# facebookresearch/robust-dynrf

Hardware: AMD Instinct MI355X
Metric: training rays/sec (Nvidia Balloon1, configs/Nvidia.txt, static+dynamic TensorVMSplit) (higher is better)
Workload: dtype f32; 1 GPU; BASELINE.json configs[1]: Nvidia Balloon1, configs/Nvidia.txt, 4096 rays/iter/GPU, 1xMI355X per rank, static+dynamic TensorVMSplit; one step = 5 dynamic + 5 static forward passes, scene-flow MLP, induced flow/disparity, per-frame depth loss, distortion loss, compositor, factor regularisers, full backward, Adam; config=nvidia, stage=stage0, samples_per_ray=115, global_batch=4096, rays_per_gpu=4096, parallelism=ray-sharded dp1, ranks=1, dead_work=executed (work the reference also computes although nothing consumes it)

## Files before the change

robust-dynrf_amd/csrc/rdrf_bwd.hip:

```cpp
#ifdef RDRF_GROWS_TEMPORAL
#define RDRF_SAVE_TEMPORAL
#endif
#include "rdrf_kernels.hpp"
#ifdef RDRF_NO_BIAS_ATOMICS
#define BIAS_ATOMIC(p, v) ((void)0)
#else
#define BIAS_ATOMIC(p, v) grad_add(p, v)
#endif

namespace pkb {
constexpr int K1H_DEN2 = 0;
constexpr int K1H_BLE2 = K1H_DEN2 + 64;
#ifdef RDRF_HEADS_BWD_F32
constexpr int K1H_DEN1T_F = K1H_BLE2 + 64;
constexpr int K1H_DEN1T_X0 = K1H_DEN1T_F + 3 * 32 * 64;
constexpr int K1H_BLE1T_F = K1H_DEN1T_X0 + 2 * 32 * 64;
constexpr int K1H_BLE1T_X0 = K1H_BLE1T_F + 3 * 32 * 64;
constexpr int K1H_SIZE = K1H_BLE1T_X0 + 2 * 32 * 64;
#else
constexpr int K1H_DEN1T_F = K1H_BLE2 + 64;
constexpr int K1H_DEN1T_X0 = K1H_DEN1T_F + 3 * 32 * 96;
constexpr int K1H_BLE1T_F = K1H_DEN1T_X0 + 2 * 32 * 96;
constexpr int K1H_BLE1T_X0 = K1H_BLE1T_F + 3 * 32 * 96;
constexpr int K1H_SIZE = K1H_BLE1T_X0 + 2 * 32 * 96;
#endif
constexpr int K1W_W5 = 0;
#ifdef RDRF_HEADS_BWD_F32
constexpr int K1W_W4T = K1W_W5 + 3 * 64;
constexpr int K1W_W3T_X0 = K1W_W4T + 2 * 32 * 64;
constexpr int K1W_W3T_T = K1W_W3T_X0 + 2 * 32 * 64;
constexpr int K1W_SIZE = K1W_W3T_T + 1 * 32 * 64;
#else
constexpr int K1W_W4T = K1W_W5 + 3 * 64;
constexpr int K1W_W3T_X0 = K1W_W4T + 2 * 32 * 96;
constexpr int K1W_W3T_T = K1W_W3T_X0 + 2 * 32 * 96;
constexpr int K1W_SIZE = K1W_W3T_T + 1 * 32 * 96;
#endif
constexpr int K3_RGBV = 0;
constexpr int K3_RGB2T = K3_RGBV + 3 * 128;
constexpr int K3_RGB1T_F = K3_RGB2T + 4 * 64 * 64;
constexpr int K3_RGB1T_X0 = K3_RGB1T_F + 1 * 64 * 64;
constexpr int K3_BASIST = K3_RGB1T_X0 + 2 * 64 * 64;
constexpr int K3_SIZE = K3_BASIST + 7 * 16 * 64;
constexpr int S3_W3 = 0;
constexpr int S3_W2T = S3_W3 + 3 * 128;
constexpr int S3_W1T_F = S3_W2T + 4 * 64 * 64;
constexpr int S3_W1T_P = S3_W1T_F + 1 * 64 * 64;
constexpr int S3_BASIST = S3_W1T_P + 4 * 64 * 64;
constexpr int S3_SIZE = S3_BASIST + 3 * 16 * 64;
constexpr int SF_W6 = 0;
constexpr int SF_W4T = SF_W6 + 6 * 64;
constexpr int SF_W2T = SF_W4T + 2 * 32 * 64;
constexpr int SF_W0T = SF_W2T + 2 * 32 * 64;
constexpr int SF_SIZE = SF_W0T + 2 * 32 * 64;
constexpr int REG_K1H = 0, REG_K1W = REG_K1H + K1H_SIZE, REG_K3 = REG_K1W + K1W_SIZE,
              REG_SF = REG_K3 + K3_SIZE, REG_DYN_END = REG_SF + SF_SIZE;
constexpr int REG_S3 = 0, REG_STAT_END = S3_SIZE;
constexpr int K3_LO_RGB2T = 0;
constexpr int K3_LO_RGB1T = K3_LO_RGB2T + 4 * 64 * 32;
constexpr int K3_LO_BASIST = K3_LO_RGB1T + 3 * 64 * 32;
constexpr int K3_LO_SIZE = K3_LO_BASIST + 7 * 16 * 32;
constexpr int S3_LO_W2T = 0;
constexpr int S3_LO_W1T = S3_LO_W2T + 4 * 64 * 32;
constexpr int S3_LO_BASIST = S3_LO_W1T + 5 * 64 * 32;
constexpr int S3_LO_SIZE = S3_LO_BASIST + 3 * 16 * 32;
constexpr int REG_K3_LO = REG_DYN_END, REG_S3_LO = REG_STAT_END;
static_assert(K3_RGB1T_X0 == K3_RGB1T_F + 64 * 64 && S3_W1T_P == S3_W1T_F + 64 * 64, "layer-1 blocks form one image");
static_assert(K1H_SIZE * 4 <= 160 * 1024 && K3_SIZE * 4 <= 160 * 1024 && S3_SIZE * 4 <= 160 * 1024,
              "backward weight images must fit the LDS");
}


#define DFS_FLOATS 144
RDRF_HD constexpr int dfs_off(int Q) {
  return (Q % 6) < 4 ? (Q / 6) * 16 + 4 * (Q % 6) : ((Q % 6) == 4 ? 48 + 4 * (Q / 6) : 60 + 4 * (Q / 6));
}

#define DFA_FLOATS 216
RDRF_HD constexpr int dfa_off(int Q) {
  return (Q % 18) < 12 ? (Q / 18) * 48 + 4 * (Q % 18)
                       : ((Q % 18) < 15 ? 144 + 12 * (Q / 18) + 4 * ((Q % 18) - 12) : 180 + 12 * (Q / 18) + 4 * ((Q % 18) - 15));
}

struct BwdArgs {
  const float* rays;
  const float* ts;
  const float* xyz;
  const float* z;
  const uint8_t* valid;
  int N, S;
  Box box;
  float distance_scale, weight_thres, density_shift;
  int act, ray_type, static_head;
  const float *g_rgb, *g_sigma, *g_weight, *g_dists, *g_blending, *g_xyz_prime;
  SavedPtrs sp;
  const float* pk;
  float* grows1;
  float* grows3;
  float* dxw_app;
  float* dxn_app;
  float* dtout;
  float* dfs;
  float* dfa;
  float* g_xyz;
  float* g_rays;
  float* g_z;
  int M, in_norm;
  const float* g_feat;
  int small_dw;
  int dynq;
};

struct StaticG {
  RdrfVM density, app;
  float *b3, *w3;
};
struct DynG {
  RdrfVM density, blending, app;
  float *rbv, *rwv, *l5b, *db2, *bb2;
  float *l5w, *dw2, *bw2;
};

template <int CTRL, int ROW_MASK = 0xF>
RDRF_D float dppf(float v) {
  if constexpr (ROW_MASK == 0xF)
    return __int_as_float(__builtin_amdgcn_update_dpp(0, __float_as_int(v), CTRL, 0xF, 0xF, true));
  else
    return __int_as_float(__builtin_amdgcn_update_dpp(__float_as_int(v), __float_as_int(v), CTRL, ROW_MASK, 0xF, false));
}
template <int CTRL, int ROW_MASK = 0xF>
RDRF_D int dppi(int v) {
  if constexpr (ROW_MASK == 0xF)
    return __builtin_amdgcn_update_dpp(0, v, CTRL, 0xF, 0xF, true);
  else
    return __builtin_amdgcn_update_dpp(v, v, CTRL, ROW_MASK, 0xF, false);
}

template <int K>
RDRF_D void atomic_quad_k(float* base, unsigned off, float val, int c) {
  constexpr int QP = K * 0x55;
  const unsigned o = (unsigned)dppi<QP>((int)off);
  if (__ballot(o != 0xffffffffu) == 0ull) return;
  if (o != 0xffffffffu) grad_add(base + (size_t)o + c, val);
}
RDRF_D void atomic_add4(float* p_base, size_t p_off, f32x4 v, bool ok) {
#if defined(RDRF_ABL_NOATOM) || defined(RDRF_ABL_NOGLOBAL)
  return;
#endif
  if (__ballot(ok) == 0ull) return;
  const int lane = threadIdx.x, c = lane & 3;
  const bool a = lane & 1, b = lane & 2;
  const float px = dppf<0xB1>(v.x), py = dppf<0xB1>(v.y), pz = dppf<0xB1>(v.z), pw = dppf<0xB1>(v.w);
  const float n0 = a ? py : v.x, n1 = a ? v.y : px, n2 = a ? pw : v.z, n3 = a ? v.w : pz;
  const float q0 = dppf<0x4E>(n0), q1 = dppf<0x4E>(n1), q2 = dppf<0x4E>(n2), q3 = dppf<0x4E>(n3);
  const float t0 = b ? q2 : n0, t1 = b ? q3 : n1, t2 = b ? n2 : q0, t3 = b ? n3 : q1;
  const unsigned off = ok ? (unsigned)p_off : 0xffffffffu;
  atomic_quad_k<0>(p_base, off, t0, c);
  atomic_quad_k<1>(p_base, off, t1, c);
  atomic_quad_k<2>(p_base, off, t2, c);
  atomic_quad_k<3>(p_base, off, t3, c);
}
RDRF_D float dot4(f32x4 a, f32x4 b) { return a.x * b.x + a.y * b.y + a.z * b.z + a.w * b.w; }

struct Run {
  int start;
  bool tail;
};
RDRF_D Run run_of(int key, int s) {
  const int prev = dppi<0x138>(key);
  const bool head = (s == 0) || (prev != key);
  const unsigned long long b = __ballot(head);
  const unsigned m = (unsigned)(b >> (32 * ((threadIdx.x & 63) >> 5)));
  Run r;
  r.start = 31 - __clz((int)(m & (0xffffffffu >> (31 - s))));
  r.tail = (s == 31) || ((m >> (s + 1)) & 1u);
  return r;
}
RDRF_D f32x4 run_scan4(f32x4 v, int start, int s) {
#ifdef RDRF_ABL_NOSCAN
  return v;
#endif
  const int sr = s & 15;
#define RDRF_SCAN_STEP(D)                                                                   \
  {                                                                                         \
// ... 768 lines not shown
  const int lane = threadIdx.x;
  const int n = blockIdx.x;
  if (n >= a.N) return;
  float vx, vy, vz;
  const float nrm = ray_norm(a.rays, n, a.ray_type, vx, vy, vz);
  if (a.g_weight) {
    float carry = 1.0f;
    for (int j0 = 0; j0 < a.S; j0 += 64) {
      if (lane == 0) carr[j0 >> 6] = carry;
      const int j = j0 + lane;
      const bool act = j < a.S;
      const int idx = n * a.S + (act ? j : 0);
      const bool vld = act && a.valid[idx] != 0;
      const float sigma = vld ? density_act(a.sp.raw[idx], a.act, a.density_shift) : 0.f;
      const float zj = act ? a.z[idx] : 0.f;
      const float zn = (j + 1 < a.S) ? a.z[idx + 1] : zj;
      const float ds = ((j + 1 < a.S) ? (zn - zj) : 0.0f) * nrm * a.distance_scale;
      const float alpha = 1.0f - expf(-sigma * ds);
      const float p = act ? one_minus_alpha_eps(alpha) : 1.0f;
      carry *= __shfl(scan_mul64(p, lane), 63, 64);
    }
  }
  __syncthreads();
  float sufcarry = 0.f, g_nrm = 0.f;
  const int ntile = (a.S + 63) >> 6;
  for (int tl = ntile - 1; tl >= 0; --tl) {
    const int j0 = tl << 6;
    const int j = j0 + lane;
    const bool act = j < a.S;
    const int idx = n * a.S + (act ? j : 0);
    const bool vld = act && a.valid[idx] != 0;
    const float f = a.sp.raw[idx];
    const float sigma = vld ? density_act(f, a.act, a.density_shift) : 0.f;
    const float zj = act ? a.z[idx] : 0.f;
    const float zn = (j + 1 < a.S) ? a.z[idx + 1] : zj;
    const float ds = ((j + 1 < a.S) ? (zn - zj) : 0.0f) * nrm * a.distance_scale;
    const float alpha = 1.0f - expf(-sigma * ds);
    const float p = act ? one_minus_alpha_eps(alpha) : 1.0f;
    float g_alpha = 0.f;
    if (a.g_weight) {
      const float incl = scan_mul64(p, lane);
      float excl = __shfl_up(incl, 1, 64);
      if (lane == 0) excl = 1.0f;
      const float T = carr[tl] * excl;
      const float gwv = act ? a.g_weight[idx] : 0.f;
      float rinc = gwv * alpha * T;
#pragma unroll
      for (int d = 1; d < 64; d <<= 1) {
        const float o = __shfl_down(rinc, d, 64);
        if (lane + d < 64) rinc += o;
      }
      float rex = __shfl_down(rinc, 1, 64);
      if (lane == 63) rex = 0.f;
      g_alpha = gwv * T - (sufcarry + rex) / p;
      sufcarry += __shfl(rinc, 0, 64);
    }
    float g_sigma = (act && a.g_sigma) ? a.g_sigma[idx] : 0.f;
    g_sigma += g_alpha * ds * (1.0f - alpha);
    if ((a.g_rays || a.g_z) && act) {
      const float g_ds = (a.g_dists ? a.g_dists[idx] : 0.f) + g_alpha * sigma * (1.0f - alpha);
      if (a.g_rays) g_nrm += g_ds * ((j + 1 < a.S) ? (zn - zj) : 0.0f) * a.distance_scale;
      if (a.g_z && j + 1 < a.S) {
        const float gz = g_ds * nrm * a.distance_scale;
        atomicAdd(a.g_z + idx, -gz);
        atomicAdd(a.g_z + idx + 1, gz);
      }
    }
    const float gf = vld ? g_sigma * act_grad(f, a.act, a.density_shift) : 0.f;
    if (act) gf_rows[(size_t)n * (((a.S + 31) >> 5) << 5) + j] = gf;
  }
  if (a.g_rays && a.ray_type != RDRF_RAY_OTHER) {
    g_nrm = wave_sum(g_nrm);
    if (lane < 3) atomicAdd(a.g_rays + (size_t)n * 6 + 3 + lane, g_nrm * (lane == 0 ? vx : (lane == 1 ? vy : vz)));
  }
}

#ifndef SC_LINES_MAX_BYTES
#define SC_LINES_MAX_BYTES (152 * 1024)
#endif
struct ScatterArgs {
  RdrfVM vm[2], gvm[2];
  int nsets;
  const float* rows;
  int stride, row0[2];
  const float* xw;
  const float* xyz;
  Box box;
  const int* list;
  const int* count;
  const uint8_t* valid;
  int N, S;
  float* dxw;
  int dxw_accumulate;
  float* g_xyz;
  int lds_bytes;
  int lds_f64;
  int bcast;
};

template <int C0Q, int C1Q, int NQ>
__global__ __launch_bounds__(512, 3) void k_scatter(ScatterArgs a) {
  extern __shared__ __attribute__((aligned(16))) float lacc[];
  const int nl0 = lines_floats(a.vm[0]), nl1 = a.nsets > 1 ? lines_floats(a.vm[1]) : 0;
  const bool use_lacc = a.lds_bytes > 0;
  if (use_lacc)
    for (int i = threadIdx.x; i < (nl0 + nl1) * (a.lds_f64 ? 2 : 1); i += blockDim.x) lacc[i] = 0.f;
  __syncthreads();
  const int lane = threadIdx.x & 63, h = lane >> 5, s = lane & 31;
  const int wave = threadIdx.x >> 6, nwaves = blockDim.x >> 6;
  const int tpr = (a.S + 31) >> 5;
  const int count = a.list ? *a.count : 0;
  const int ntiles = a.list ? ((count + 31) >> 5) : a.N * tpr;
  for (int t = blockIdx.x * nwaves + wave; t < ntiles; t += gridDim.x * nwaves) {
    int idx;
    bool live;
    if (a.list) {
      const int li = t * 32 + s;
      live = li < count;
      idx = live ? a.list[li] : 0;
    } else {
      const int n = t / tpr, j = (t - n * tpr) * 32 + s;
      const bool act = j < a.S;
      idx = n * a.S + (act ? j : 0);
      live = act && a.valid[idx] != 0;
    }
    float x0, x1, x2;
    if (a.xw) {
      x0 = a.xw[(size_t)idx * 3 + 0]; x1 = a.xw[(size_t)idx * 3 + 1]; x2 = a.xw[(size_t)idx * 3 + 2];
    } else {
      x0 = norm_c(a.xyz[(size_t)idx * 3 + 0], a.box.lo[0], a.box.inv[0]);
      x1 = norm_c(a.xyz[(size_t)idx * 3 + 1], a.box.lo[1], a.box.inv[1]);
      x2 = norm_c(a.xyz[(size_t)idx * 3 + 2], a.box.lo[2], a.box.inv[2]);
    }
    const float xa0 = __shfl(x0, lane & 15, 64), xa1 = __shfl(x1, lane & 15, 64), xa2 = __shfl(x2, lane & 15, 64);
    const float xb0 = __shfl(x0, 16 + (lane & 15), 64), xb1 = __shfl(x1, 16 + (lane & 15), 64),
                xb2 = __shfl(x2, 16 + (lane & 15), 64);
    const bool livea = __shfl((int)live, lane & 15, 64) != 0, liveb = __shfl((int)live, 16 + (lane & 15), 64) != 0;
    float dw0 = 0.f, dw1 = 0.f, dw2 = 0.f;
    for (int set = 0; set < a.nsets; ++set) {
      const float* rb = a.rows + ((size_t)t * a.stride + a.row0[set]) * 32;
      const LdsLines ll = make_lds_lines(use_lacc ? lacc : nullptr, set ? nl0 : 0, a.lds_f64, a.vm[set]);
#ifndef RDRF_SC_UNROLL
#define RDRF_SC_UNROLL 1
#endif
      constexpr bool ZSPLIT = C0Q <= 4;
      constexpr int QPL = C0Q + 2 * C1Q, NLV = (2 * NQ) / QPL;
      static_assert(C0Q % 4 == 0 && NLV * QPL == 2 * NQ, "quad layout");
      const int q = lane >> 4, s16 = lane & 15;
#ifndef RDRF_ABL_SC_NLV
#define RDRF_ABL_SC_NLV 99
#endif
#pragma unroll 1
      for (int lv = 0; lv < NLV && lv < RDRF_ABL_SC_NLV; ++lv) {
#ifndef RDRF_ABL_SC_NOXY
#pragma unroll 1
        for (int it = 0; it < C0Q / 2; ++it) {
          const int grp = it >> 1, j = it & 1;
          const int g = lv * QPL + 4 * grp + q;
          const int sidx = 16 * j + s16;
          const float* rq = rb + (a.bcast ? (size_t)0 : (size_t)(4 * g) * 32) + sidx;
          const int rs = a.bcast ? 0 : 32;
          const f32x4 dq = {rq[0], rq[rs], rq[2 * rs], rq[3 * rs]};
          gather_xy4_bwd<C0Q, C1Q>(a.vm[set], a.gvm[set], lv, 4 * grp + q, j ? xb0 : xa0, j ? xb1 : xa1,
                                   j ? xb2 : xa2, dq, j ? liveb : livea, lane < 32 && q == j, dw0, dw1, dw2, ll);
        }
#endif
#ifndef RDRF_ABL_SC_NOZ
        if constexpr (ZSPLIT) {
#pragma unroll 1
          for (int zq = 0; zq < 2 * C1Q; ++zq) {
            const int g = lv * QPL + C0Q + zq;
            const float* rq = rb + (a.bcast ? (size_t)0 : (size_t)(4 * g) * 32) + s;
            const int rs = a.bcast ? 0 : 32;
            const f32x4 dq = {rq[0], rq[rs], rq[2 * rs], rq[3 * rs]};
            gather_zquad_bwd<C0Q, C1Q>(a.vm[set], a.gvm[set], g, h, x0, x1, x2, dq, live, s, dw0, dw1, dw2, ll);
          }
        } else {
#pragma unroll 1
          for (int zp = 0; zp < C1Q; ++zp) {
            const int g = lv * QPL + C0Q + 2 * zp + h;
            const float* rq = rb + (a.bcast ? (size_t)0 : (size_t)(4 * g) * 32) + s;
            const int rs = a.bcast ? 0 : 32;
            const f32x4 dq = {rq[0], rq[rs], rq[2 * rs], rq[3 * rs]};
            gather_quad_bwd<C0Q, C1Q, 1>(a.vm[set], a.gvm[set], g, x0, x1, x2, dq, live, s, dw0, dw1, dw2, ll);
          }
        }
#endif
      }
    }
    dw0 += __shfl_xor(dw0, 32, 64); dw1 += __shfl_xor(dw1, 32, 64); dw2 += __shfl_xor(dw2, 32, 64);
    if (live && h == 0) {
      if (a.dxw) {
        float* d = a.dxw + (size_t)idx * 3;
        if (a.dxw_accumulate) { d[0] += dw0; d[1] += dw1; d[2] += dw2; }
        else { d[0] = dw0; d[1] = dw1; d[2] = dw2; }
      }
      if (a.g_xyz) {
        a.g_xyz[(size_t)idx * 3 + 0] += dw0 * a.box.inv[0];
        a.g_xyz[(size_t)idx * 3 + 1] += dw1 * a.box.inv[1];
        a.g_xyz[(size_t)idx * 3 + 2] += dw2 * a.box.inv[2];
      }
    }
  }
  if (use_lacc) {
    __syncthreads();
    flush_lds_lines(lacc, a.lds_f64, 0, a.vm[0], a.gvm[0]);
    if (a.nsets > 1) flush_lds_lines(lacc, a.lds_f64, nl0, a.vm[1], a.gvm[1]);
  }
}

struct SortKeyArgs {
  const float* xw;
  const uint8_t* valid;
  const float* grows1;
  const int* list;
  const int* count;
  int N, S;
  int W[3], H[3];
  int kb;
  unsigned* keys;
  int* counts;
  int compact;
};

RDRF_D int cell_axis(float c, int L, bool& any) {
  const Tap1 t0 = tap1d(c, L), t1 = tap1d(c, (L + 1) >> 1), t2 = tap1d(c, (L + 3) >> 2);
  any = t0.ok0 || t0.ok1 || t1.ok0 || t1.ok1 || t2.ok0 || t2.ok1;
  return min(max(t0.i0, -2), L) + 2;
}

__global__ __launch_bounds__(256) void k_sort_keys(SortKeyArgs a) {
  const int NS = a.N * a.S, tpr = (a.S + 31) >> 5;
  const int count = a.list ? *a.count : 0;
  const int nent = (a.list && a.compact) ? count : NS;
  for (int e = blockIdx.x * blockDim.x + threadIdx.x; e < nent; e += gridDim.x * blockDim.x) {
    bool live = false;
    float x0 = 0.f, x1 = 0.f, x2 = 0.f;
    if (a.list) {
      live = e < count;
      const int idx = live ? a.list[e] : 0;
      x0 = a.xw[(size_t)idx * 3 + 0]; x1 = a.xw[(size_t)idx * 3 + 1]; x2 = a.xw[(size_t)idx * 3 + 2];
    } else {
      const int idx = e;
      const int n = idx / a.S, j = idx - n * a.S;
      const float* sm = a.grows1 + ((size_t)(n * tpr + (j >> 5)) * sv::K1G_ROWS + sv::K1G_SM) * 32 + (j & 31);
      live = a.valid[idx] != 0 && (sm[3 * 32] != 0.f || sm[4 * 32] != 0.f);
      x0 = a.xw[(size_t)idx * 3 + 0]; x1 = a.xw[(size_t)idx * 3 + 1]; x2 = a.xw[(size_t)idx * 3 + 2];
    }
#pragma unroll
    for (int p = 0; p < 3; ++p) {
      const float cx = p == 2 ? x1 : x0, cy = p == 0 ? x1 : x2;
      bool ax, ay;
      const int ix = cell_axis(cx, a.W[p], ax), iy = cell_axis(cy, a.H[p], ay);
      const bool in = live && ax && ay;
      const unsigned cell = in ? (unsigned)(iy * (a.W[p] + 3) + ix) : ((1u << a.kb) - 1u);
      a.keys[(size_t)p * nent + e] = ((unsigned)p << a.kb) | cell;
    }
  }
}

__global__ void k_sort_counts(const unsigned* __restrict__ keys_sorted, int NS, int kb, int* __restrict__ counts,
                              const int* __restrict__ seg) {
  const int p = threadIdx.x;
  if (p >= 3) return;
  const int stride = seg ? *seg : NS;
  const unsigned drop = ((unsigned)p << kb) | ((1u << kb) - 1u);
  const unsigned* k = keys_sorted + (size_t)p * stride;
  int lo = 0, hi = stride;
  while (lo < hi) {
    const int mid = (lo + hi) >> 1;
    if (k[mid] < drop) lo = mid + 1; else hi = mid;
  }
  counts[p] = lo;
}

#ifndef RDRF_LINE_DIRECT_DEFAULT
#define RDRF_LINE_DIRECT_DEFAULT 1
#endif
struct SortedScatterArgs {
  RdrfVM vm[2], gvm[2];
  int set_mask;
  const unsigned* order;
  const int* count;
  unsigned base;
  const int* seg;
  const float* dfs;
  int rec_floats;
  const int* list;
  const float* xw;
  float* dxw;
  int lds_bytes, lds_f64;
  int line_direct;
  const unsigned* keys;
  int kb, Wk, tw, slice_steps, tile_sets;
};

template <int PLANE, int C0Q, int C1Q>
__global__ __launch_bounds__(512, 3) void k_scatter_sorted(SortedScatterArgs a) {
  extern __shared__ __attribute__((aligned(16))) float lacc[];
  const int nl0 = (a.set_mask & 1) ? a.vm[0].L[PLANE] * lds_stride(a.vm[0].C[PLANE]) : 0;
  const int nl1 = (a.set_mask & 2) ? a.vm[1].L[PLANE] * lds_stride(a.vm[1].C[PLANE]) : 0;
  const bool use_lacc = a.lds_bytes > 0;
  if (use_lacc)
    for (int i = threadIdx.x; i < (nl0 + nl1) * (a.lds_f64 ? 2 : 1); i += blockDim.x) lacc[i] = 0.f;
  __syncthreads();
  const int lane = threadIdx.x & 63, h = lane >> 5, s = lane & 31, q = lane >> 4, s16 = lane & 15;
  const int wave = threadIdx.x >> 6, nwaves = blockDim.x >> 6;
  const int count = *a.count;
  const unsigned obase = a.seg ? (unsigned)PLANE * (unsigned)*a.seg : a.base;
  const unsigned* order = a.seg ? a.order + obase : a.order;
  constexpr int SPT = PLANE == 0 ? 16 : 32;
  constexpr int XYF = 4 * C0Q, ZF = 4 * C1Q, SETF = 3 * XYF + 6 * ZF, QPL = C0Q + 2 * C1Q;
  const int ntiles = (count + SPT - 1) / SPT;
  for (int t = blockIdx.x * nwaves + wave; t < ntiles; t += gridDim.x * nwaves) {
    const int pos = t * SPT + (PLANE == 0 ? s16 : s);
    const bool live = pos < count;
    const int ent = live ? (int)(order[pos] - obase) : 0;
    const int idx = a.list ? a.list[ent] : ent;
    const float x0 = a.xw[(size_t)idx * 3 + 0], x1 = a.xw[(size_t)idx * 3 + 1], x2 = a.xw[(size_t)idx * 3 + 2];
    float dw0 = 0.f, dw1 = 0.f, dw2 = 0.f;
#pragma unroll 1
    for (int set = 0; set < 2; ++set) {
      if (!((a.set_mask >> set) & 1)) continue;
      const int first = set ? nl0 : 0;
      const LdsLines ll = LdsLines{use_lacc ? lacc : nullptr, {first, first, first}, a.lds_f64, a.line_direct};
      const float* rec = a.dfs + (size_t)ent * a.rec_floats + set * SETF;
#pragma unroll 1
      for (int lv = 0; lv < 3; ++lv) {
// ... 72 lines not shown
    }
    __syncthreads();
    for (int t = wave; t * SPT < e_hi - e_lo; t += nwaves) {
      const int pos = e_lo + t * SPT + (PLANE == 0 ? s16 : s);
      const bool live = pos < e_hi;
      const int ent = live ? (int)(a.order[pos] - a.base) : 0;
      const int idx = a.list ? a.list[ent] : ent;
      const float x0 = a.xw[(size_t)idx * 3 + 0], x1 = a.xw[(size_t)idx * 3 + 1], x2 = a.xw[(size_t)idx * 3 + 2];
      float dw0 = 0.f, dw1 = 0.f, dw2 = 0.f;
#pragma unroll 1
      for (int set = 0; set < 2; ++set) {
        if (!((a.set_mask >> set) & 1)) continue;
        const int first = set ? nl0 : 0;
        const LdsLines ll = LdsLines{lacc, {first, first, first}, 1, a.line_direct};
        const int tslot = set == 1 && (a.set_mask & 1) ? 1 : 0;
        const PlaneTile T = PlaneTile{lacc + 2 * (nl0 + nl1 + tslot * tile_elems), s_geo, CT};
        const float* rec = a.dfs + (size_t)ent * a.rec_floats + set * SETF;
#pragma unroll 1
        for (int lv = 0; lv < 3; ++lv) {
          if constexpr (PLANE == 0) {
#pragma unroll 1
            for (int grp = 0; grp < C0Q / 4; ++grp) {
              const f32x4 dq = live ? ld4(rec + lv * XYF + grp * 16 + 4 * q) : f32x4{0.f, 0.f, 0.f, 0.f};
              gather_xy4_bwd<C0Q, C1Q, true>(a.vm[set], a.gvm[set], lv, 4 * grp + q, x0, x1, x2, dq, live, q == 0, dw0, dw1, dw2, ll, T);
            }
          } else {
#pragma unroll 1
            for (int zq = 0; zq < C1Q; ++zq) {
              const f32x4 dq = live ? ld4(rec + 3 * XYF + (PLANE - 1) * 3 * ZF + lv * ZF + 4 * zq) : f32x4{0.f, 0.f, 0.f, 0.f};
              gather_zquad_bwd<C0Q, C1Q, true>(a.vm[set], a.gvm[set], lv * QPL + C0Q + (PLANE - 1) * C1Q + zq, h, x0, x1, x2, dq, live, s,
                                               dw0, dw1, dw2, ll, T);
            }
          }
        }
      }
      if constexpr (PLANE != 0) {
        dw0 += __shfl_xor(dw0, 32, 64); dw1 += __shfl_xor(dw1, 32, 64); dw2 += __shfl_xor(dw2, 32, 64);
      }
      if (live && (PLANE == 0 ? q == 0 : h == 0)) {
        float* d = a.dxw + (size_t)idx * 3;
        d[0] += dw0; d[1] += dw1; d[2] += dw2;
      }
    }
    __syncthreads();
#pragma unroll 1
    for (int set = 0; set < 2; ++set) {
      if (!((a.set_mask >> set) & 1)) continue;
      double* tile = reinterpret_cast<double*>(lacc) + nl0 + nl1 + (set == 1 && (a.set_mask & 1) ? 1 : 0) * tile_elems;
      float* GP = a.gvm[set].plane[PLANE];
      const int sH = a.vm[set].sH[PLANE], sW = a.vm[set].sW[PLANE];
      for (int lv = 0; lv < 3; ++lv) {
        const int gx0 = s_geo[lv * 8 + 0], gy0 = s_geo[lv * 8 + 1], nx = s_geo[lv * 8 + 2], ny = s_geo[lv * 8 + 3], off = s_geo[lv * 8 + 4];
        const int n = nx * ny * CT;
        for (int i = threadIdx.x; i < n; i += blockDim.x) {
          const double v = tile[off + i];
          if (v != 0.0) {
            tile[off + i] = 0.0;
            const int t = i / CT, cc = i - t * CT, ty = t / nx, tx = t - ty * nx;
            grad_add(GP + (size_t)(((gy0 + ty) << lv) * sH + ((gx0 + tx) << lv) * sW) + cc, (float)v);
          }
        }
      }
    }
  }
  __syncthreads();
  if (a.set_mask & 1) flush_lds_line(lacc, 1, 0, a.vm[0].L[PLANE], a.vm[0].C[PLANE], a.gvm[0].line[PLANE]);
  if (a.set_mask & 2) flush_lds_line(lacc, 1, nl0, a.vm[1].L[PLANE], a.vm[1].C[PLANE], a.gvm[1].line[PLANE]);
}

RDRF_D float reduce_scatter32(const float (&p)[32], int s) {
  const bool b4 = s & 16, b3 = s & 8, b2 = s & 4, b1 = s & 2, b0 = s & 1;
  float q[16], r[8], t[4], u[2];
#pragma unroll
  for (int i = 0; i < 16; ++i) q[i] = (b4 ? p[i + 16] : p[i]) + __shfl_xor(b4 ? p[i] : p[i + 16], 16, 64);
#pragma unroll
  for (int i = 0; i < 8; ++i) r[i] = (b3 ? q[i + 8] : q[i]) + __shfl_xor(b3 ? q[i] : q[i + 8], 8, 64);
#pragma unroll
  for (int i = 0; i < 4; ++i) t[i] = (b2 ? r[i + 4] : r[i]) + __shfl_xor(b2 ? r[i] : r[i + 4], 4, 64);
#pragma unroll
  for (int i = 0; i < 2; ++i) u[i] = (b1 ? t[i + 2] : t[i]) + __shfl_xor(b1 ? t[i] : t[i + 2], 2, 64);
  return (b0 ? u[1] : u[0]) + __shfl_xor(b0 ? u[0] : u[1], 1, 64);
}

template <int PHASE, bool FEAT>
__global__ __launch_bounds__(64 * RDRF_MAXW) void k_dyn_density_bwd(BwdArgs a, DynW w, DynG gw) {
  __shared__ __attribute__((aligned(16))) float lds[PHASE == 0 ? pkb::K1H_SIZE : pkb::K1W_SIZE];
  __shared__ float carr[8][128];
  lds_fill(lds, a.pk + (PHASE == 0 ? pkb::REG_K1H : pkb::REG_K1W), PHASE == 0 ? pkb::K1H_SIZE : pkb::K1W_SIZE);
  const int lane = threadIdx.x & 63, h = lane >> 5, s = lane & 31;
  const int wave = threadIdx.x >> 6, nwaves = blockDim.x >> 6;
  const int tpr = (a.S + 31) >> 5;
  float sw[3] = {0.f, 0.f, 0.f}, sb[3] = {0.f, 0.f, 0.f};
  for (int n = blockIdx.x * nwaves + wave; n < a.N; n += gridDim.x * nwaves) {
    float vx = 0.f, vy = 0.f, vz = 0.f;
    float nrm = 1.0f;
    if constexpr (!FEAT) nrm = ray_norm(a.rays, n, a.ray_type, vx, vy, vz);
    if (!FEAT && PHASE == 0 && a.g_weight) {
      float carry = 1.0f;
      for (int j0 = 0; j0 < a.S; j0 += 32) {
        if (lane == 0) carr[wave][j0 >> 5] = carry;
        const int j = j0 + s;
        const bool act = j < a.S;
        const int idx = n * a.S + (act ? j : 0);
        const bool vld = act && a.valid[idx] != 0;
        const float sigma = vld ? density_act(a.sp.raw[(size_t)idx * 2], a.act, a.density_shift) : 0.f;
        const float zj = act ? a.z[idx] : 0.f;
        const float zn = (j + 1 < a.S) ? a.z[idx + 1] : zj;
        const float ds = ((j + 1 < a.S) ? (zn - zj) : 0.0f) * nrm * a.distance_scale;
        const float alpha = 1.0f - expf(-sigma * ds);
        const float p = act ? one_minus_alpha_eps(alpha) : 1.0f;
        carry *= __shfl(scan_mul32(p, s), 31, 32);
      }
    }
    float sufcarry = 0.f, g_nrm = 0.f;
    float dTacc[16];
#pragma unroll
    for (int i = 0; i < 16; ++i) dTacc[i] = 0.f;
    for (int tli = tpr - 1; tli >= 0; --tli) {
      const int j0 = tli << 5;
      const int j = j0 + s;
      const bool act = j < a.S && (!FEAT || n * a.S + j < a.M);
      const int idx = n * a.S + (act ? j : 0);
      const bool vld = act && (FEAT || a.valid[idx] != 0);
      const size_t tl = (size_t)n * tpr + tli;
      const float* svb = a.sp.act1 + tl * sv::K1_ROWS * 32;
      float* gb = a.grows1 + tl * sv::K1G_ROWS * 32;
      if (PHASE == 0) {
        float g_fd, g_fb;
        if constexpr (FEAT) {
          g_fd = (act && a.g_sigma) ? a.g_sigma[idx] : 0.f;
          g_fb = (act && a.g_blending) ? a.g_blending[idx] : 0.f;
        } else {
        const float fd = a.sp.raw[(size_t)idx * 2], fb = a.sp.raw[(size_t)idx * 2 + 1];
        const float sigma = vld ? density_act(fd, a.act, a.density_shift) : 0.f;
        const float zj = act ? a.z[idx] : 0.f;
        const float zn = (j + 1 < a.S) ? a.z[idx + 1] : zj;
        const float ds = ((j + 1 < a.S) ? (zn - zj) : 0.0f) * nrm * a.distance_scale;
        const float alpha = 1.0f - expf(-sigma * ds);
        const float p = act ? one_minus_alpha_eps(alpha) : 1.0f;
        float g_alpha = 0.f;
        if (a.g_weight) {
          const float incl = scan_mul32(p, s);
          float excl = __shfl_up(incl, 1, 32);
          if (s == 0) excl = 1.0f;
          const float T = carr[wave][tli] * excl;
          const float gwv = act ? a.g_weight[idx] : 0.f;
          float rinc = gwv * alpha * T;
#pragma unroll
          for (int d = 1; d < 32; d <<= 1) {
            const float o = __shfl_down(rinc, d, 32);
            if (s + d < 32) rinc += o;
          }
          float rex = __shfl_down(rinc, 1, 32);
          if (s == 31) rex = 0.f;
          g_alpha = gwv * T - (sufcarry + rex) / p;
          sufcarry += __shfl(rinc, 0, 32);
        }
        float g_sigma = (act && a.g_sigma) ? a.g_sigma[idx] : 0.f;
        g_sigma += g_alpha * ds * (1.0f - alpha);
        if ((a.g_rays || a.g_z) && act && h == 0) {
          const float g_ds = (a.g_dists ? a.g_dists[idx] : 0.f) + g_alpha * sigma * (1.0f - alpha);
          if (a.g_rays) g_nrm += g_ds * ((j + 1 < a.S) ? (zn - zj) : 0.0f) * a.distance_scale;
          if (a.g_z && j + 1 < a.S) {
            const float gz = g_ds * nrm * a.distance_scale;
            atomicAdd(a.g_z + idx, -gz);
            atomicAdd(a.g_z + idx + 1, gz);
          }
        }
        g_fd = vld ? g_sigma * act_grad(fd, a.act, a.density_shift) : 0.f;
        const float bl = sigmoidf_(fb);
        g_fb = (vld && a.g_blending) ? a.g_blending[idx] * bl * (1.0f - bl) : 0.f;
        }
        f32x16 accX[2];
        acc_zero<2>(accX);
        const bool live_d = FEAT ? a.g_sigma != nullptr : (a.g_sigma != nullptr || a.g_weight != nullptr);
        const bool live_b = a.g_blending != nullptr;
#pragma unroll
        for (int head = 0; head < 2; ++head) {
          if (!(head == 0 ? live_d : live_b)) continue;
          const float gfh = head == 0 ? g_fd : g_fb;
          float Hh[32], dzh[32];
          load_rows<32>(svb, head == 0 ? sv::K1_HD : sv::K1_HB, Hh, s, h);
          const float* w2 = lds + (head == 0 ? pkb::K1H_DEN2 : pkb::K1H_BLE2) + h * 32;
          float w2r[32];
#pragma unroll
          for (int q = 0; q < 8; ++q) {
            const f32x4 v = *reinterpret_cast<const f32x4*>(w2 + 4 * q);
            w2r[4 * q] = v.x; w2r[4 * q + 1] = v.y; w2r[4 * q + 2] = v.z; w2r[4 * q + 3] = v.w;
          }
#pragma unroll
          for (int kk = 0; kk < 32; ++kk) dzh[kk] = Hh[kk] > 0.f ? w2r[kk] * gfh : 0.f;
          save_rows<32>(gb, head == 0 ? sv::K1G_DZD : sv::K1G_DZB, dzh, s, h);
          if (!FEAT && a.small_dw) {
            float pw[32];
#pragma unroll
            for (int kk = 0; kk < 32; ++kk) pw[kk] = gfh * Hh[kk];
            sw[head] += reduce_scatter32(pw, s);
            sb[head] += gfh;
          }
          f32x16 accF[3];
          acc_zero<3>(accF);
#ifdef RDRF_HEADS_BWD_F32
          mfma_seg<3, 32>(accF, dzh, lds + (head == 0 ? pkb::K1H_DEN1T_F : pkb::K1H_BLE1T_F), lane);
          mfma_seg<2, 32>(accX, dzh, lds + (head == 0 ? pkb::K1H_DEN1T_X0 : pkb::K1H_BLE1T_X0), lane);
#else
          mfma_seg_b3_pair<3, 2, 32>(accF, accX, dzh, lds + (head == 0 ? pkb::K1H_DEN1T_F : pkb::K1H_BLE1T_F),
                                     lds + (head == 0 ? pkb::K1H_DEN1T_X0 : pkb::K1H_BLE1T_X0), lane);
#endif
          float dFh[48];
          acc_copy<3>(dFh, accF);
          if (!FEAT && a.dfs != nullptr) {
            if (act) {
              float* rec = a.dfs + (size_t)idx * DFS_FLOATS + head * 72;
#pragma unroll
// ... 45 lines not shown
              const float d = wa[c] * dd0 + wb[c] * dd1 + wc[c] * dd2;
              dz4[4 * q + c] = H4[4 * q + c] > 0.f ? d : 0.f;
            }
          }
          if (!FEAT && a.small_dw) {
            sb[0] += dd0; sb[1] += dd1; sb[2] += dd2;
#pragma unroll 1
            for (int o = 0; o < 3; ++o) {
              const float dd = o == 0 ? dd0 : (o == 1 ? dd1 : dd2);
              float pw[32];
#pragma unroll
              for (int kk = 0; kk < 32; ++kk) pw[kk] = dd * H4[kk];
              const float r = reduce_scatter32(pw, s);
              sw[0] += o == 0 ? r : 0.f; sw[1] += o == 1 ? r : 0.f; sw[2] += o == 2 ? r : 0.f;
            }
          }
        }
        save_rows<32>(gb, sv::K1G_DZ4, dz4, s, h);
        float dz3[32];
        {
          f32x16 acc[2];
          acc_zero<2>(acc);
#ifdef RDRF_HEADS_BWD_F32
          mfma_seg<2, 32>(acc, dz4, lds + pkb::K1W_W4T, lane);
#else
          mfma_seg_b3<2, 32>(acc, dz4, lds + pkb::K1W_W4T, lane);
#endif
          float H3[32];
          load_rows<32>(svb, sv::K1_H3, H3, s, h);
#pragma unroll
          for (int kk = 0; kk < 32; ++kk) dz3[kk] = H3[kk] > 0.f ? acc[kk >> 4][kk & 15] : 0.f;
        }
        save_rows<32>(gb, sv::K1G_DZ3, dz3, s, h);
        f32x16 accX[2];
        {
          float dXh[32];
          load_rows<32>(gb, sv::K1G_DX0, dXh, s, h);
#pragma unroll
          for (int kk = 0; kk < 32; ++kk) accX[kk >> 4][kk & 15] = dXh[kk];
        }
#ifdef RDRF_HEADS_BWD_F32
        mfma_seg<2, 32>(accX, dz3, lds + pkb::K1W_W3T_X0, lane);
#endif
        {
          f32x16 accT[1];
          acc_zero<1>(accT);
#ifdef RDRF_HEADS_BWD_F32
          mfma_seg<1, 32>(accT, dz3, lds + pkb::K1W_W3T_T, lane);
#else
          mfma_seg_b3_pair<2, 1, 32>(accX, accT, dz3, lds + pkb::K1W_W3T_X0, lds + pkb::K1W_W3T_T, lane);
#endif
#pragma unroll
          for (int i = 0; i < 16; ++i) dTacc[i] += accT[0][i];
        }
        {
          float X0[32], dX0[32];
          load_rows<32>(svb, sv::K1_X0, X0, s, h);
          acc_copy<2>(dX0, accX);
          float e0 = 0.f, e1 = 0.f, e2 = 0.f;
          x0_bwd(X0, dX0, h, e0, e1, e2);
          e0 += __shfl_xor(e0, 32, 64); e1 += __shfl_xor(e1, 32, 64); e2 += __shfl_xor(e2, 32, 64);
          dn0 += e0 + dw0; dn1 += e1 + dw1; dn2 += e2 + dw2;
        }
        if (act && h == 0 && a.g_xyz) {
          if (FEAT && a.in_norm) {
            a.g_xyz[(size_t)idx * 3 + 0] += dn0; a.g_xyz[(size_t)idx * 3 + 1] += dn1;
            a.g_xyz[(size_t)idx * 3 + 2] += dn2;
          } else {
            a.g_xyz[(size_t)idx * 3 + 0] += dn0 * a.box.inv[0] + gp0;
            a.g_xyz[(size_t)idx * 3 + 1] += dn1 * a.box.inv[1] + gp1;
            a.g_xyz[(size_t)idx * 3 + 2] += dn2 * a.box.inv[2] + gp2;
          }
        }
        if constexpr (FEAT) {
          if (act) {
#pragma unroll
            for (int i = 0; i < 16; ++i) a.dtout[(size_t)idx * 32 + elem_of(i, h)] = dTacc[i];
          }
#pragma unroll
          for (int i = 0; i < 16; ++i) dTacc[i] = 0.f;
        }
      }
    }
    if (PHASE == 1 && !FEAT) {
#pragma unroll
      for (int i = 0; i < 16; ++i) {
        float v = dTacc[i];
#pragma unroll
        for (int d = 16; d >= 1; d >>= 1) v += __shfl_xor(v, d, 64);
        if (s == 0) a.dtout[(size_t)n * 32 + elem_of(i, h)] = v;
      }
    }
    if (!FEAT && PHASE == 0 && a.g_rays && a.ray_type != RDRF_RAY_OTHER) {
      g_nrm = wave_sum(g_nrm);
      if (lane < 3) atomicAdd(a.g_rays + (size_t)n * 6 + 3 + lane, g_nrm * (lane == 0 ? vx : (lane == 1 ? vy : vz)));
    }
  }
  if (!FEAT && a.small_dw) {
    __shared__ float red[8][3][65];
    __syncthreads();
#pragma unroll
    for (int o = 0; o < 3; ++o) {
      red[wave][o][lane] = sw[o];
      const float bs = wave_sum(h == 0 ? sb[o] : 0.f);
      if (lane == 0) red[wave][o][64] = bs;
    }
    __syncthreads();
    if (wave == 0) {
      const bool live_d = a.g_sigma != nullptr || a.g_weight != nullptr, live_b = a.g_blending != nullptr;
#pragma unroll
      for (int o = 0; o < 3; ++o) {
        float v = 0.f, bv = 0.f;
        for (int wv = 0; wv < nwaves; ++wv) { v += red[wv][o][lane]; bv += red[wv][o][64]; }
        float* gwt = PHASE == 1 ? gw.l5w + o * 64 : (o == 0 ? gw.dw2 : gw.bw2);
        float* gbs = PHASE == 1 ? gw.l5b + o : (o == 0 ? gw.db2 : gw.bb2);
        const bool on = PHASE == 1 ? true : (o == 0 ? live_d : (o == 1 ? live_b : false));
        if (on) {
          grad_add(gwt + elem_of(s, h), v);
          if (lane == 0) grad_add(gbs, bv);
        }
      }
    }
  }
}

#define TB_RPB 32
__global__ __launch_bounds__(128) void k_time_branch_bwd(const float* __restrict__ ts, DynW w, int N,
                                                         const float* __restrict__ dtout,
                                                         float* __restrict__ g_l1w,
                                                         float* __restrict__ g_l1b,
                                                         float* __restrict__ g_l2w,
                                                         float* __restrict__ g_l2b) {
  __shared__ float s_tin[TB_RPB][17];
  __shared__ float s_h[TB_RPB][65];
  __shared__ float s_dz1[TB_RPB][65];
  __shared__ float s_dz2[TB_RPB][31];
  const int tid = threadIdx.x;
  const int r = tid >> 2, q = tid & 3;
  const int n = blockIdx.x * TB_RPB + r;
  const bool act = n < N;
  float tin[17];
  const float t = act ? ts[n] : 0.f;
  tin[0] = t;
#pragma unroll
  for (int f = 0; f < 8; ++f) sincosf(ldexpf(t, f), &tin[1 + f], &tin[9 + f]);
  if (q == 0)
    for (int i = 0; i < 17; ++i) s_tin[r][i] = tin[i];
  for (int o = q; o < 30; o += 4) s_dz2[r][o] = act ? dtout[(size_t)n * 32 + o] : 0.f;
  __syncthreads();
  for (int k = 16 * q; k < 16 * q + 16; ++k) {
    float hk = w.l1b[k];
#pragma unroll
    for (int i = 0; i < 17; ++i) hk = fmaf(w.l1w[k * 17 + i], tin[i], hk);
    float dh = 0.f;
    for (int o = 0; o < 30; ++o) dh = fmaf(w.l2w[o * 64 + k], s_dz2[r][o], dh);
    s_h[r][k] = fmaxf(hk, 0.f);
    s_dz1[r][k] = hk > 0.f ? dh : 0.f;
  }
  __syncthreads();
  for (int e = tid; e < 30 * 64; e += 128) {
    const int o = e / 64, k = e - o * 64;
    float a = 0.f;
    for (int rr = 0; rr < TB_RPB; ++rr) a = fmaf(s_dz2[rr][o], s_h[rr][k], a);
    grad_add(g_l2w + e, a);
  }
  for (int e = tid; e < 64 * 17; e += 128) {
    const int k = e / 17, i = e - k * 17;
    float a = 0.f;
    for (int rr = 0; rr < TB_RPB; ++rr) a = fmaf(s_dz1[rr][k], s_tin[rr][i], a);
    grad_add(g_l1w + e, a);
  }
  if (tid < 30) {
    float a = 0.f;
    for (int rr = 0; rr < TB_RPB; ++rr) a += s_dz2[rr][tid];
    grad_add(g_l2b + tid, a);
  }
  if (tid < 64) {
    float a = 0.f;
    for (int rr = 0; rr < TB_RPB; ++rr) a += s_dz1[rr][tid];
    grad_add(g_l1b + tid, a);
  }
}

RDRF_D void sf_x_bwd(const float (&X)[20], const float (&dX)[20], int h, float& d0, float& d1,
                     float& d2) {
#pragma unroll
  for (int o = 0; o < 5; ++o) {
    if (o == 0 && h == 0) {
      d0 += dX[0]; d1 += dX[1]; d2 += dX[2];
    } else {
      const int k = 2 * o + h - 1;
#pragma unroll
      for (int p = 0; p < 2; ++p) {
        const int pr = 2 * k + p;
        if (pr < 12) {
          const int d = pr >> 2, f = pr & 3;
          const float dq = ldexpf(dX[o * 4 + 2 * p] * X[o * 4 + 2 * p + 1] -
                                  dX[o * 4 + 2 * p + 1] * X[o * 4 + 2 * p], f);
          d0 += d == 0 ? dq : 0.f; d1 += d == 1 ? dq : 0.f; d2 += d == 2 ? dq : 0.f;
        }
      }
    }
  }
}

__global__ __launch_bounds__(64 * RDRF_MAXW) void k_scene_flow_bwd(int N, int S, Box box,
                                                        const float* __restrict__ pkg,
                                                        const float* __restrict__ act_rows,
                                                        float* __restrict__ grows,
                                                        const float* __restrict__ g_f,
                                                        const float* __restrict__ g_b,
                                                        float* __restrict__ g_sfb6,
                                                        float* __restrict__ g_pts) {
  __shared__ __attribute__((aligned(16))) float lds[pkb::SF_SIZE];
  lds_fill(lds, pkg + pkb::REG_SF, pkb::SF_SIZE);
  const int lane = threadIdx.x & 63, h = lane >> 5, s = lane & 31;
  const int wave = threadIdx.x >> 6, nwaves = blockDim.x >> 6;
  const int total = N * S;
  const int ntiles = (total + 31) >> 5;
  for (int tile = blockIdx.x * nwaves + wave; tile < ntiles; tile += gridDim.x * nwaves) {
    const int li = tile * 32 + s;
    const bool act = li < total;
    const int idx = act ? li : 0;
    const float* svb = act_rows + (size_t)tile * sv::SF_ROWS * 32;
    float* gb = grows + (size_t)tile * sv::SFG_ROWS * 32;
    float dz6[6];
#pragma unroll
    for (int o = 0; o < 6; ++o) {
      const float* gsrc = o < 3 ? g_f : g_b;
      dz6[o] = (act && gsrc) ? gsrc[(size_t)idx * 3 + (o % 3)] : 0.f;
      if (h == 0) gb[(size_t)(sv::SFG_DZ6 + o) * 32 + s] = dz6[o];
// ... 489 lines not shown
#endif
  pack_add(J, P->dw1, 152, 64, 72, SEG_IDENT, hm, 3, 32, kh + K1H_DEN1T_F);
  pack_add(J, P->dw1, 152, 64, 152, SEG_DEN1_X0, hm, 2, 32, kh + K1H_DEN1T_X0);
  pack_add(J, P->bw1, 152, 64, 72, SEG_IDENT, hm, 3, 32, kh + K1H_BLE1T_F);
  pack_add(J, P->bw1, 152, 64, 152, SEG_DEN1_X0, hm, 2, 32, kh + K1H_BLE1T_X0);
  pack_add(J, P->rwv, 131, 3, 128, SEG_IDENT, 1, 3, 64, k3 + K3_RGBV);
#ifdef RDRF_APP_F32
  pack_add(J, P->rw2, 128, 128, 128, SEG_IDENT, 2, 4, 64, k3 + K3_RGB2T);
  pack_add(J, P->rw1, 107, 128, 107, SEG_RGB1_F, 2, 1, 64, k3 + K3_RGB1T_F);
  pack_add(J, P->rw1, 107, 128, 107, SEG_RGB1_X0, 2, 2, 64, k3 + K3_RGB1T_X0);
  pack_add(J, P->basis, 216, 27, 216, SEG_IDENT, 2, 7, 16, k3 + K3_BASIST);
#else
  pack_add_b3s_t(J, P->rw2, 128, 128, 128, SEG_IDENT, 4, 64, k3 + K3_RGB2T, REG_K3_LO + K3_LO_RGB2T);
  pack_add_b3s_t(J, P->rw1, 107, 128, 107, SEG_RGB1_F, 1, 64, k3 + K3_RGB1T_F, REG_K3_LO + K3_LO_RGB1T);
  pack_add_b3s_t(J, P->rw1, 107, 128, 107, SEG_RGB1_X0, 2, 64, k3 + K3_RGB1T_X0, REG_K3_LO + K3_LO_RGB1T + 64 * 32);
  pack_add_b3s_t(J, P->basis, 216, 27, 216, SEG_IDENT, 7, 16, k3 + K3_BASIST, REG_K3_LO + K3_LO_BASIST);
#endif
  pack_add(J, P->sfw[3], 64, 6, 64, SEG_IDENT, 1, 6, 32, sf + SF_W6);
  pack_add(J, P->sfw[2], 64, 64, 64, SEG_IDENT, 2, 2, 32, sf + SF_W4T);
  pack_add(J, P->sfw[1], 64, 64, 64, SEG_IDENT, 2, 2, 32, sf + SF_W2T);
  pack_add(J, P->sfw[0], 36, 64, 36, SEG_SF_X, 2, 2, 32, sf + SF_W0T);
}

static void static_pack_jobs_bwd(PackJobs& J, const RdrfStaticParams* P, int head) {
  using namespace pkb;
  J.n = 0;
  const bool fea = head == RDRF_HEAD_MLP_FEA;
  const int in1 = fea ? 138 : 135;
  pack_add(J, P->w3, fea ? 128 : 131, 3, 128, SEG_IDENT, 1, 3, 64, REG_S3 + S3_W3);
#ifdef RDRF_APP_F32
  pack_add(J, P->w2, 128, 128, 128, SEG_IDENT, 2, 4, 64, REG_S3 + S3_W2T);
  pack_add(J, P->w1, in1, 128, in1, fea ? SEG_STAT1_F_FEA : SEG_STAT1_F_TE, 2, 1, 64, REG_S3 + S3_W1T_F);
  pack_add(J, P->w1, in1, 128, in1, fea ? SEG_STAT1_P_FEA : SEG_STAT1_P_TE, 2, 4, 64, REG_S3 + S3_W1T_P);
  pack_add(J, P->basis, 72, 27, 72, SEG_IDENT, 2, 3, 16, REG_S3 + S3_BASIST);
#else
  pack_add_b3s_t(J, P->w2, 128, 128, 128, SEG_IDENT, 4, 64, REG_S3 + S3_W2T, REG_S3_LO + S3_LO_W2T);
  pack_add_b3s_t(J, P->w1, in1, 128, in1, fea ? SEG_STAT1_F_FEA : SEG_STAT1_F_TE, 1, 64, REG_S3 + S3_W1T_F, REG_S3_LO + S3_LO_W1T);
  pack_add_b3s_t(J, P->w1, in1, 128, in1, fea ? SEG_STAT1_P_FEA : SEG_STAT1_P_TE, 4, 64, REG_S3 + S3_W1T_P, REG_S3_LO + S3_LO_W1T + 64 * 32);
  pack_add_b3s_t(J, P->basis, 72, 27, 72, SEG_IDENT, 3, 16, REG_S3 + S3_BASIST, REG_S3_LO + S3_LO_BASIST);
#endif
}

struct Geo {
  int grid, block;
};
static Geo geo_for_units(long units) {
  Geo g;
  const int ncu = 256;
  int waves = (int)((units + ncu - 1) / ncu);
  waves = waves < 1 ? 1 : (waves > RDRF_MAXW ? RDRF_MAXW : waves);
  g.block = waves * 64;
  long blocks = (units + waves - 1) / waves;
  g.grid = (int)(blocks < 1 ? 1 : (blocks > ncu ? ncu : blocks));
  return g;
}

#define PACK_AREA_FLOATS (1 << 20)
static_assert(pkb::REG_K3_LO + pkb::K3_LO_SIZE <= PACK_AREA_FLOATS && pkb::REG_S3_LO + pkb::S3_LO_SIZE <= PACK_AREA_FLOATS,
              "the backward images and their streamed lo pieces fit the pack area");

static void fill_bwd_common(BwdArgs& a, const RdrfFieldCfg* cfg, const float* rays, const float* ts,
                            const float* xyz, const float* z, const uint8_t* valid, int N, int S) {
  memset(&a, 0, sizeof(a));
  a.rays = rays; a.ts = ts; a.xyz = xyz; a.z = z; a.valid = valid; a.N = N; a.S = S;
  a.box = make_box(cfg);
  a.distance_scale = cfg->distance_scale; a.weight_thres = cfg->weight_thres;
  a.density_shift = cfg->density_shift; a.act = cfg->act; a.ray_type = cfg->ray_type;
  a.static_head = cfg->static_head;
  static const int dynq = RDRF_ENV("RDRF_DYNQ") ? atoi(RDRF_ENV("RDRF_DYNQ")) : 1;
  a.dynq = dynq;
}

extern "C" size_t rdrf_forward_workspace_bytes(int N, int S) {
  const size_t ns = (size_t)N * S;
  return (size_t)PACK_AREA_FLOATS * 4 + 256 + (size_t)N * 32 * 4 + ns * 3 * 4 + ns * 4 + (1 << 12);
}

extern "C" size_t rdrf_workspace_bytes(int N, int S) {
  size_t ns = (size_t)N * S, t1 = (size_t)N * ((S + 31) / 32), t3 = (ns + 31) / 32;
  size_t fwd = rdrf_forward_workspace_bytes(N, S);
  size_t bwd = (size_t)PACK_AREA_FLOATS * 4 + t1 * sv::K1G_ROWS * 32 * 4 + t3 * sv::K3G_ROWS * 32 * 4 +
               ns * 3 * 4 * 2 + (size_t)N * 32 * 4 + (1 << 14);
  bwd += ns * DFS_FLOATS * 4 + ns * DFA_FLOATS * 4 + 3 * ns * 4 * 3 + 1024 + rdrf_sort_temp_bytes((unsigned)(3 * ns), 32) + (1 << 12);
  size_t sf = (size_t)PACK_AREA_FLOATS * 4 + t3 * sv::SFG_ROWS * 32 * 4 + (1 << 12);
  size_t m = fwd > bwd ? fwd : bwd;
  return m > sf ? m : sf;
}

struct BwdWs {
  float* dfs;
  float* dfa;
  unsigned *keys_in, *keys_out, *order;
  int* counts;
  void* sort_tmp;
  size_t sort_tmp_bytes;
  float* pk;
  float* gf;
  float* grows1;
  float* grows3;
  float* dxw;
  float* dxn;
  float* dtout;
};
static int carve_bwd(BwdWs& b, void* ws, size_t ws_bytes, int N, int S, int dynamic) {
  WsCarver c(ws, ws_bytes);
  size_t ns = (size_t)N * S, t1 = (size_t)N * ((S + 31) / 32), t3 = (ns + 31) / 32;
  b.pk = c.take<float>(PACK_AREA_FLOATS);
  b.grows3 = c.take<float>(t3 * sv::K3G_ROWS * 32);
  b.grows1 = dynamic ? c.take<float>(t1 * sv::K1G_ROWS * 32) : nullptr;
  b.dxw = dynamic ? c.take<float>(ns * 3) : nullptr;
  b.dxn = dynamic ? c.take<float>(ns * 3) : nullptr;
  b.dtout = dynamic ? c.take<float>((size_t)N * 32) : nullptr;
  b.gf = dynamic ? nullptr : c.take<float>(t1 * 32);
  b.dfs = nullptr;
  b.dfa = nullptr;
  if (dynamic) {
    b.dfs = c.take<float>(ns * DFS_FLOATS);
    b.dfa = c.take<float>(ns * DFA_FLOATS);
    b.keys_in = c.take<unsigned>(3 * ns);
    b.keys_out = c.take<unsigned>(3 * ns);
    b.order = c.take<unsigned>(3 * ns);
    b.counts = c.take<int>(64);
    b.sort_tmp_bytes = rdrf_sort_temp_bytes((unsigned)(3 * ns), 32);
    b.sort_tmp = c.take<char>(b.sort_tmp_bytes);
  }
  RDRF_CHECK(c.ok(), -3, "backward workspace too small: need %zu have %zu", c.off, ws_bytes);
  return 0;
}

static void fill_scatter_common(ScatterArgs& sa, const BwdArgs& a) {
  memset(&sa, 0, sizeof(sa));
  sa.xyz = a.xyz; sa.box = a.box; sa.valid = a.valid; sa.N = a.N; sa.S = a.S;
}
static int lines_floats_host(const RdrfVM& vm) {
  int n = 0;
  for (int i = 0; i < 3; ++i) n += vm.L[i] * (vm.C[i] + 4);
  return n;
}
#ifndef RDRF_SC_THREADS2_DEFAULT
#define RDRF_SC_THREADS2_DEFAULT 256
#endif
template <typename K>
static int launch_scatter(const char* name, K kern, ScatterArgs& sa, long ntiles, hipStream_t stream) {
  const long n0 = lines_floats_host(sa.vm[0]), n1 = sa.nsets > 1 ? lines_floats_host(sa.vm[1]) : 0;
  static const int f64_env = RDRF_ENV("RDRF_LDS_F64") ? atoi(RDRF_ENV("RDRF_LDS_F64")) : 1;
  int esz = 0;
  bool split = false;
  for (int e = f64_env ? 8 : 4; e >= 4 && !esz; e -= 4) {
    if (e * (n0 + n1) <= SC_LINES_MAX_BYTES) esz = e;
    else if (sa.nsets == 2 && e * n0 <= SC_LINES_MAX_BYTES && e * n1 <= SC_LINES_MAX_BYTES) { esz = e; split = true; }
  }
#ifdef RDRF_DETERMINISTIC
  esz = 0;
  split = false;
#endif
  if (split) {
    ScatterArgs s0 = sa, s1 = sa;
    s0.nsets = 1;
    s1.nsets = 1;
    s1.vm[0] = sa.vm[1]; s1.gvm[0] = sa.gvm[1]; s1.row0[0] = sa.row0[1];
    s1.dxw_accumulate = 1;
    int rc = launch_scatter(name, kern, s0, ntiles, stream);
    return rc ? rc : launch_scatter(name, kern, s1, ntiles, stream);
  }
  sa.lds_bytes = (int)(esz * (n0 + n1));
  sa.lds_f64 = esz == 8;
  if (sa.lds_bytes > 48 * 1024)
    RDRF_HIP(hipFuncSetAttribute((const void*)kern, hipFuncAttributeMaxDynamicSharedMemorySize, SC_LINES_MAX_BYTES));
  const int per_cu = sa.lds_bytes > 80 * 1024 ? 1 : (sa.lds_bytes > 53 * 1024 ? 2 : 3);
  static const int thr2_env = RDRF_ENV("RDRF_SC_THREADS2") ? atoi(RDRF_ENV("RDRF_SC_THREADS2")) : RDRF_SC_THREADS2_DEFAULT;
  const int threads = per_cu == 1 ? 512 : (per_cu == 2 ? thr2_env : 256);
  const int wpb = threads / 64;
  long g = (ntiles + wpb - 1) / wpb;
  static const long cap_env = RDRF_ENV("RDRF_SC_CAP") ? atol(RDRF_ENV("RDRF_SC_CAP")) : 0;
  const long cap = per_cu == 1 ? 256 : (cap_env > 0 ? cap_env : 256 * per_cu);
  g = g < 1 ? 1 : (g > cap ? cap : g);
  rdrf_prof_begin(name, stream);
  hipLaunchKernelGGL(kern, dim3((unsigned)g), dim3(threads), (size_t)sa.lds_bytes, stream, sa);
  rdrf_prof_end(name, stream);
  RDRF_HIP(hipGetLastError());
  return 0;
}

static int g_scatter_mode = RDRF_SCATTER_AUTO;
extern "C" int rdrf_set_scatter_mode(int mode) {
  RDRF_CHECK(mode == RDRF_SCATTER_AUTO || mode == RDRF_SCATTER_RAY || mode == RDRF_SCATTER_SORTED || mode == RDRF_SCATTER_SORTED_PLAIN, -1,
             "rdrf_set_scatter_mode: mode must be RDRF_SCATTER_AUTO, _RAY, _SORTED or _SORTED_PLAIN");
  g_scatter_mode = mode;
  return 0;
}
static int scatter_mode(size_t ns, hipStream_t stream) {
  int m = g_scatter_mode;
  if (const char* e = RDRF_ENV("RDRF_SCATTER")) m = !strcmp(e, "sorted") ? RDRF_SCATTER_SORTED : (!strcmp(e, "ray") ? RDRF_SCATTER_RAY : m);
  if (m == RDRF_SCATTER_AUTO) {
    hipStreamCaptureStatus cs = hipStreamCaptureStatusNone;
    if (hipStreamIsCapturing(stream, &cs) == hipSuccess && cs == hipStreamCaptureStatusActive) return 1;
    return ns >= (size_t)300000 ? 1 : 0;
  }
  return (m == RDRF_SCATTER_SORTED || m == RDRF_SCATTER_SORTED_PLAIN) ? 1 : 0;
}

template <int PLANE, int C0Q, int C1Q>
static int launch_scatter_sorted(SortedScatterArgs& sa, long max_samples, hipStream_t stream) {
  const long n = ((sa.set_mask & 1) ? (long)sa.vm[0].L[PLANE] * (sa.vm[0].C[PLANE] + 4) : 0) +
                 ((sa.set_mask & 2) ? (long)sa.vm[1].L[PLANE] * (sa.vm[1].C[PLANE] + 4) : 0);
  static const int f64_env = RDRF_ENV("RDRF_LDS_F64") ? atoi(RDRF_ENV("RDRF_LDS_F64")) : 1;
  const int esz = (f64_env && 8 * n <= SC_LINES_MAX_BYTES) ? 8 : (4 * n <= SC_LINES_MAX_BYTES ? 4 : 0);
// ... 76 lines not shown
  rdrf_prof_end(names[PLANE], stream);
  RDRF_HIP(hipGetLastError());
  return 1;
}

static int sorted_scatter_prepare(SortKeyArgs& ka, const RdrfVM& vm, const BwdArgs& a, const BwdWs& b, hipStream_t stream) {
  const size_t ns = (size_t)a.N * a.S;
  ka.xw = a.sp.xw; ka.valid = a.valid; ka.N = a.N; ka.S = a.S;
  long maxcells = 0;
  for (int p = 0; p < 3; ++p) {
    ka.W[p] = vm.W[p]; ka.H[p] = vm.H[p];
    const long c = (long)(ka.W[p] + 3) * (ka.H[p] + 3);
    maxcells = c > maxcells ? c : maxcells;
  }
  int kb = 1;
  while (((1L << kb) - 1) < maxcells) ++kb;
  RDRF_CHECK(kb <= 29, -1, "sorted scatter: plane too large for 32-bit keys");
  ka.kb = kb; ka.keys = b.keys_in; ka.counts = b.counts;
  rdrf_prof_begin("scatter_sort", stream);
  {
    long g = ((long)ns + 255) / 256;
    g = g > 2048 ? 2048 : g;
    rdrf_prof_begin("sort_keys", stream);
    hipLaunchKernelGGL(k_sort_keys, dim3((unsigned)g), dim3(256), 0, stream, ka);
    rdrf_prof_end("sort_keys", stream);
  }
  int rc = rdrf_sort_positions(b.keys_in, b.keys_out, b.order, (unsigned)(3 * ns), kb + 2, b.sort_tmp, b.sort_tmp_bytes, stream,
                               ka.compact ? ka.count : nullptr, 3u);
  if (rc) return rc;
  hipLaunchKernelGGL(k_sort_counts, dim3(1), dim3(64), 0, stream, (const unsigned*)b.keys_out, (int)ns, kb, b.counts,
                     ka.compact ? ka.count : (const int*)nullptr);
  rdrf_prof_end("scatter_sort", stream);
  RDRF_HIP(hipGetLastError());
  return 0;
}

static int scatter_dyn_app_sorted(const BwdArgs& a, const BwdWs& b, const RdrfDynamicParams* P, const RdrfDynamicParams* G,
                                  hipStream_t stream) {
  const size_t ns = (size_t)a.N * a.S;
  SortKeyArgs ka;
  memset(&ka, 0, sizeof(ka));
  ka.list = a.sp.list; ka.count = &a.sp.hdr->count;
#ifdef RDRF_TOOLS
  static const int compact_env = RDRF_ENV("RDRF_SORT_COMPACT") ? atoi(RDRF_ENV("RDRF_SORT_COMPACT")) : 1;
  ka.compact = compact_env && !(RDRF_ENV("RDRF_SS_TILED") && atoi(RDRF_ENV("RDRF_SS_TILED")) >= 2);
#else
  ka.compact = 1;
#endif
  int rc = sorted_scatter_prepare(ka, P->app, a, b, stream);
  if (rc) return rc;
  SortedScatterArgs sa;
  memset(&sa, 0, sizeof(sa));
  sa.vm[0] = P->app; sa.gvm[0] = G->app;
  sa.set_mask = 1; sa.dfs = b.dfa; sa.rec_floats = DFA_FLOATS; sa.list = a.sp.list; sa.xw = a.sp.xw; sa.dxw = b.dxw;
  for (int p = 0; p < 3; ++p) {
    sa.order = b.order + (size_t)p * ns; sa.count = b.counts + p; sa.base = (unsigned)(p * ns);
    if (ka.compact) { sa.order = b.order; sa.seg = ka.count; }
    const unsigned* ks = b.keys_out + (size_t)p * ns;
#ifdef RDRF_TOOLS
    rc = p == 0 ? launch_scatter_tiled<0, 12, 3>(sa, ks, ka.kb, (long)ns, stream)
                : (p == 1 ? launch_scatter_tiled<1, 12, 3>(sa, ks, ka.kb, (long)ns, stream)
                          : launch_scatter_tiled<2, 12, 3>(sa, ks, ka.kb, (long)ns, stream));
    if (rc < 0) return rc;
    if (rc == 1) continue;
#else
    (void)ks;
#endif
    rc = p == 0 ? launch_scatter_sorted<0, 12, 3>(sa, (long)ns, stream)
                : (p == 1 ? launch_scatter_sorted<1, 12, 3>(sa, (long)ns, stream) : launch_scatter_sorted<2, 12, 3>(sa, (long)ns, stream));
    if (rc) return rc;
  }
  return 0;
}

static int scatter_dyn_density_sorted(const BwdArgs& a, const BwdWs& b, const RdrfDynamicParams* P, const RdrfDynamicParams* G,
                                      int set_mask, hipStream_t stream) {
  const size_t ns = (size_t)a.N * a.S;
  for (int p = 0; p < 3; ++p)
    RDRF_CHECK(P->blending.W[p] == P->density.W[p] && P->blending.H[p] == P->density.H[p], -1,
               "sorted scatter: density and blending planes differ in size");
  SortKeyArgs ka;
  memset(&ka, 0, sizeof(ka));
  ka.grows1 = b.grows1;
  int rc = sorted_scatter_prepare(ka, P->density, a, b, stream);
  if (rc) return rc;
  SortedScatterArgs sa;
  memset(&sa, 0, sizeof(sa));
  sa.vm[0] = P->density; sa.gvm[0] = G->density; sa.vm[1] = P->blending; sa.gvm[1] = G->blending;
  sa.set_mask = set_mask; sa.dfs = b.dfs; sa.rec_floats = DFS_FLOATS; sa.xw = a.sp.xw; sa.dxw = b.dxw;
  for (int p = 0; p < 3; ++p) {
    sa.order = b.order + (size_t)p * ns; sa.count = b.counts + p; sa.base = (unsigned)(p * ns);
    const unsigned* ks = b.keys_out + (size_t)p * ns;
    rc = p == 0 ? launch_scatter_tiled<0, 4, 1>(sa, ks, ka.kb, (long)ns, stream)
                : (p == 1 ? launch_scatter_tiled<1, 4, 1>(sa, ks, ka.kb, (long)ns, stream)
                          : launch_scatter_tiled<2, 4, 1>(sa, ks, ka.kb, (long)ns, stream));
    if (rc < 0) return rc;
    if (rc == 1) continue;
    rc = p == 0 ? launch_scatter_sorted<0, 4, 1>(sa, (long)ns, stream)
                : (p == 1 ? launch_scatter_sorted<1, 4, 1>(sa, (long)ns, stream) : launch_scatter_sorted<2, 4, 1>(sa, (long)ns, stream));
    if (rc) return rc;
  }
  return 0;
}

static void add_density_phase_dw(DwJobs& D, const float* grows1, const float* act1, const RdrfDynamicParams* G,
                                 int T1, bool live_d = true, bool live_b = true, bool small_in_kernel = false) {
  dw_add(D, grows1, sv::K1G_ROWS, sv::K1G_DZ3, 2, 64, 0, act1, sv::K1_ROWS, 93, 93, G->l3w, G->l3b, nullptr, T1);
  dw_blk(D, sv::K1_X0, SEG_WARP3_X0, 0);
  dw_blk(D, sv::K1_X0 + 32, SEG_WARP3_X0, 32);
  dw_blk(D, sv::K1_T, SEG_WARP3_T, 0);
  dw_add(D, grows1, sv::K1G_ROWS, sv::K1G_DZ4, 2, 64, 0, act1, sv::K1_ROWS, 64, 64, G->l4w, G->l4b, nullptr, T1);
  dw_blk(D, sv::K1_H3, SEG_IDENT, 0);
  dw_blk(D, sv::K1_H3 + 32, SEG_IDENT, 32);
  if (!small_in_kernel) {
  dw_add(D, grows1, sv::K1G_ROWS, sv::K1G_SM, 1, 3, 0, act1, sv::K1_ROWS, 64, 64, G->l5w, G->l5b, nullptr, T1);
  dw_blk(D, sv::K1_H4, SEG_IDENT, 0);
  dw_blk(D, sv::K1_H4 + 32, SEG_IDENT, 32);
  if (live_d) {
    dw_add(D, grows1, sv::K1G_ROWS, sv::K1G_SM, 1, 1, 3, act1, sv::K1_ROWS, 64, 64, G->dw2, G->db2, nullptr, T1);
    dw_blk(D, sv::K1_HD, SEG_IDENT, 0);
    dw_blk(D, sv::K1_HD + 32, SEG_IDENT, 32);
  }
  if (live_b) {
    dw_add(D, grows1, sv::K1G_ROWS, sv::K1G_SM, 1, 1, 4, act1, sv::K1_ROWS, 64, 64, G->bw2, G->bb2, nullptr, T1);
    dw_blk(D, sv::K1_HB, SEG_IDENT, 0);
    dw_blk(D, sv::K1_HB + 32, SEG_IDENT, 32);
  }
  }
  for (int head = 0; head < 2; ++head) {
    if (!(head ? live_b : live_d)) continue;
    dw_add(D, grows1, sv::K1G_ROWS, head ? sv::K1G_DZB : sv::K1G_DZD, 2, 64, 0, act1, sv::K1_ROWS, 152, 152,
           head ? G->bw1 : G->dw1, head ? G->bb1 : G->db1, nullptr, T1);
    const int f0 = head ? sv::K1_FB : sv::K1_FD;
    dw_blk(D, f0, SEG_IDENT72, 0);
    dw_blk(D, f0 + 32, SEG_IDENT72, 32);
    dw_blk(D, f0 + 64, SEG_IDENT72, 64);
    dw_blk(D, sv::K1_X0, SEG_DEN1_X0, 0);
    dw_blk(D, sv::K1_X0 + 32, SEG_DEN1_X0, 32);
    dw_blk(D, sv::K1_X1, SEG_DEN1_X1, 0);
  }
}

extern "C" int rdrf_static_bwd(const RdrfStaticParams* P, const RdrfFieldCfg* cfg, const float* rays,
                               const float* ts, const float* xyz, const float* z,
                               const uint8_t* valid, int N, int S, const float* g_rgb,
                               const float* g_sigma, const float* g_weight, const float* g_dists,
                               const RdrfStaticParams* G, float* g_xyz, float* g_z, float* g_rays,
                               void* saved, size_t saved_bytes, void* ws, size_t ws_bytes,
                               rdrf_stream_t stream_) {
  hipStream_t stream = (hipStream_t)stream_;
  if (N == 0) return 0;
  RDRF_CHECK(P && cfg && G && saved && N > 0 && S > 0 && S <= 4096, -1, "static_bwd: bad arguments (S <= 4096)");
  RDRF_CHECK((size_t)N * S * 3 < (size_t)INT32_MAX, -1, "static_bwd: N * S * 3 must stay below 2^31 (32-bit sample indices)");
  BwdArgs a;
  fill_bwd_common(a, cfg, rays, ts, xyz, z, valid, N, S);
  a.g_rgb = g_rgb; a.g_sigma = g_sigma; a.g_weight = g_weight; a.g_xyz = g_xyz;
  a.g_rays = g_rays; a.g_dists = g_dists; a.g_z = g_z;
  RDRF_CHECK(carve_saved(a.sp, saved, saved_bytes, 0, N, S), -3, "static_bwd: saved buffer too small");
  BwdWs b;
  int rc = carve_bwd(b, ws, ws_bytes, N, S, 0);
  if (rc) return rc;
  a.pk = b.pk; a.grows3 = b.grows3;
  StaticW w;
  fill_static_w(w, P);
  StaticG gw;
  gw.density = G->density; gw.app = G->app; gw.b3 = G->b3; gw.w3 = G->w3;
// ... 3 lines not shown
    static_pack_jobs_bwd(J, P, cfg->static_head);
    rc = pack_launch(J, b.pk, stream);
    if (rc) return rc;
  }
  const size_t t3 = ((size_t)N * S + 31) / 32;
  if (g_rgb != nullptr) {
    const Geo g = geo_for_units((long)t3);
    if (cfg->static_head == RDRF_HEAD_MLP_FEA)
      RDRF_LAUNCH("static_app_bwd", (k_static_app_bwd<RDRF_HEAD_MLP_FEA, false>), dim3(g.grid), dim3(g.block),
                  stream, a, w, gw);
    else
      RDRF_LAUNCH("static_app_bwd", (k_static_app_bwd<RDRF_HEAD_MLP_FEA_TIMEEMBEDDING, false>), dim3(g.grid),
                  dim3(g.block), stream, a, w, gw);
    {
      ScatterArgs sa;
      fill_scatter_common(sa, a);
      sa.vm[0] = P->app; sa.gvm[0] = G->app; sa.nsets = 1;
      sa.rows = b.grows3; sa.stride = sv::K3G_ROWS; sa.row0[0] = sv::K3G_DA;
      sa.list = a.sp.list; sa.count = &a.sp.hdr->count;
      sa.g_xyz = g_xyz;
      { int rc_ = launch_scatter("scatter_static_app", k_scatter<12, 3, 9>, sa, (long)t3, stream); if (rc_) return rc_; }
    }
    const bool fea = cfg->static_head == RDRF_HEAD_MLP_FEA;
    const int in1 = fea ? 138 : 135;
    const int* cnt = &a.sp.hdr->count;
    DwJobs D;
    D.n = 0;
    dw_add(D, b.grows3, sv::K3G_ROWS, sv::K3G_DZV, 1, 3, 0, a.sp.act3, sv::S3_ROWS, 128,
           fea ? 128 : 131, G->w3, G->b3, cnt, 0);
    for (int i = 0; i < 4; ++i) dw_blk(D, sv::S3_H2 + 32 * i, SEG_IDENT, 32 * i);
    if (!fea) dw_blk(D, sv::S3_VD, SEG_VIEW3, 0);
    dw_add(D, b.grows3, sv::K3G_ROWS, sv::K3G_DF, 1, 27, 0, a.sp.act3, sv::S3_ROWS, 72, 72, G->basis,
           nullptr, cnt, 0);
    for (int i = 0; i < 3; ++i) dw_blk(D, sv::S3_G + 32 * i, SEG_IDENT, 32 * i);
    dw_add(D, b.grows3, sv::K3G_ROWS, sv::K3G_DZ2, 4, 128, 0, a.sp.act3, sv::S3_ROWS, 128, 128, G->w2,
           G->b2, cnt, 0);
    for (int i = 0; i < 4; ++i) dw_blk(D, sv::S3_H1 + 32 * i, SEG_IDENT, 32 * i);
    dw_add(D, b.grows3, sv::K3G_ROWS, sv::K3G_DZ1, 4, 128, 0, a.sp.act3, sv::S3_ROWS, in1, in1, G->w1,
           G->b1, cnt, 0);
    dw_blk(D, sv::S3_F, fea ? SEG_STAT1_F_FEA : SEG_STAT1_F_TE, 0);
    for (int i = 0; i < 4; ++i) dw_blk(D, sv::S3_P + 32 * i, fea ? SEG_STAT1_P_FEA : SEG_STAT1_P_TE, 32 * i);
    rc = dw_launch(D, stream, "dw_static");
    if (rc) return rc;
  }
  if (g_sigma != nullptr || g_weight != nullptr || ((g_rays != nullptr || g_z != nullptr) && g_dists != nullptr)) {
    RDRF_LAUNCH("static_density_bwd", k_static_density_bwd, dim3(N), dim3(64), stream, a, w, b.gf);
    if (g_sigma != nullptr || g_weight != nullptr) {
      ScatterArgs sa;
      fill_scatter_common(sa, a);
      sa.vm[0] = P->density; sa.gvm[0] = G->density; sa.nsets = 1;
      sa.rows = b.gf; sa.stride = 1; sa.row0[0] = 0; sa.bcast = 1;
      sa.g_xyz = g_xyz;
      const long t1 = (long)N * ((S + 31) / 32);
      { int rc_ = launch_scatter("scatter_static_density", k_scatter<4, 1, 3>, sa, t1, stream); if (rc_) return rc_; }
    }
  }
  return 0;
}

extern "C" int rdrf_dynamic_bwd(const RdrfDynamicParams* P, const RdrfFieldCfg* cfg,
                                const float* rays, const float* ts, const float* xyz,
                                const float* z, const uint8_t* valid, int N, int S,
                                const float* g_blending, const float* g_weight,
                                const float* g_xyz_prime, const float* g_rgb, const float* g_sigma,
                                const float* g_dists, const RdrfDynamicParams* G, float* g_xyz,
                                float* g_z, float* g_rays, void* saved, size_t saved_bytes, void* ws,
                                size_t ws_bytes, rdrf_stream_t stream_) {
  hipStream_t stream = (hipStream_t)stream_;
  if (N == 0) return 0;
  RDRF_CHECK(P && cfg && G && saved && N > 0 && S > 0 && S <= 4096, -1, "dynamic_bwd: bad arguments (S <= 4096)");
  RDRF_CHECK((size_t)N * S * 3 < (size_t)INT32_MAX, -1, "dynamic_bwd: N * S * 3 must stay below 2^31 (32-bit sample indices)");
  BwdArgs a;
  fill_bwd_common(a, cfg, rays, ts, xyz, z, valid, N, S);
  a.g_rgb = g_rgb; a.g_sigma = g_sigma; a.g_weight = g_weight; a.g_blending = g_blending;
  a.g_xyz_prime = g_xyz_prime; a.g_xyz = g_xyz; a.g_rays = g_rays; a.g_dists = g_dists; a.g_z = g_z;
  static const bool small_dw = !(RDRF_ENV("RDRF_DW_SMALL") && atoi(RDRF_ENV("RDRF_DW_SMALL")) == 0);
  a.small_dw = small_dw ? 1 : 0;
  RDRF_CHECK(carve_saved(a.sp, saved, saved_bytes, 1, N, S), -3, "dynamic_bwd: saved buffer too small");
  BwdWs b;
  int rc = carve_bwd(b, ws, ws_bytes, N, S, 1);
  if (rc) return rc;
  a.pk = b.pk; a.grows1 = b.grows1; a.grows3 = b.grows3; a.dxw_app = b.dxw; a.dxn_app = b.dxn;
  a.dtout = b.dtout;
  DynW w;
  fill_dyn_w(w, P);
  DynG gw;
  gw.density = G->density; gw.blending = G->blending; gw.app = G->app;
  gw.rbv = G->rbv; gw.rwv = G->rwv; gw.l5b = G->l5b; gw.db2 = G->db2; gw.bb2 = G->bb2;
  gw.l5w = G->l5w; gw.dw2 = G->dw2; gw.bw2 = G->bw2;
  if (P->packed_bwd != nullptr) a.pk = P->packed_bwd;
  else {
    PackJobs J;
    dyn_pack_jobs_bwd(J, P);
    rc = pack_launch(J, b.pk, stream);
    if (rc) return rc;
  }
  const size_t ns = (size_t)N * S, t3 = (ns + 31) / 32, t1 = (size_t)N * ((S + 31) / 32);
  RDRF_FILL(b.dxw, 0, ns * 3 * 4, stream);
  RDRF_FILL(b.dxn, 0, ns * 3 * 4, stream);
  const int* cnt = &a.sp.hdr->count;
  DwJobs D;
  D.n = 0;
  if (g_rgb != nullptr) {
    const Geo g = geo_for_units((long)t3);
    const int smode_app = scatter_mode(ns, stream);
    a.dfa = smode_app != 0 ? b.dfa : nullptr;
    if (smode_app != 0) RDRF_LAUNCH("dyn_app_bwd", (k_dyn_app_bwd<false, true>), dim3(g.grid), dim3(g.block), stream, a, w, gw);
    else RDRF_LAUNCH("dyn_app_bwd", (k_dyn_app_bwd<false, false>), dim3(g.grid), dim3(g.block), stream, a, w, gw);
    if (smode_app != 0) {
      rdrf_prof_begin("scatter_dyn_app", stream);
      rc = scatter_dyn_app_sorted(a, b, P, G, stream);
      rdrf_prof_end("scatter_dyn_app", stream);
      if (rc) return rc;
    } else {
      ScatterArgs sa;
      fill_scatter_common(sa, a);
      sa.vm[0] = P->app; sa.gvm[0] = G->app; sa.nsets = 1;
      sa.rows = b.grows3; sa.stride = sv::K3G_ROWS; sa.row0[0] = sv::K3G_DA;
      sa.xw = a.sp.xw; sa.list = a.sp.list; sa.count = cnt;
      sa.dxw = b.dxw; sa.dxw_accumulate = 0;
      { int rc_ = launch_scatter("scatter_dyn_app", k_scatter<12, 3, 27>, sa, (long)t3, stream); if (rc_) return rc_; }
    }
    dw_add(D, b.grows3, sv::K3G_ROWS, sv::K3G_DZV, 1, 3, 0, a.sp.act3, sv::K3_ROWS, 128, 131, G->rwv,
           G->rbv, cnt, 0);
    for (int i = 0; i < 4; ++i) dw_blk(D, sv::K3_H2 + 32 * i, SEG_IDENT, 32 * i);
    dw_blk(D, sv::K3_VD, SEG_VIEW3, 0);
    dw_add(D, b.grows3, sv::K3G_ROWS, sv::K3G_DF, 1, 27, 0, a.sp.act3, sv::K3_ROWS, 216, 216, G->basis,
           nullptr, cnt, 0);
    for (int i = 0; i < 7; ++i) dw_blk(D, sv::K3_A + 32 * i, SEG_IDENT, 32 * i);
    dw_add(D, b.grows3, sv::K3G_ROWS, sv::K3G_DZ2, 4, 128, 0, a.sp.act3, sv::K3_ROWS, 128, 128, G->rw2,
           G->rb2, cnt, 0);
    for (int i = 0; i < 4; ++i) dw_blk(D, sv::K3_H1 + 32 * i, SEG_IDENT, 32 * i);
    dw_add(D, b.grows3, sv::K3G_ROWS, sv::K3G_DZ1, 4, 128, 0, a.sp.act3, sv::K3_ROWS, 107, 107, G->rw1,
           G->rb1, cnt, 0);
    dw_blk(D, sv::K3_F, SEG_RGB1_F, 0);
    dw_blk(D, sv::K3_X0, SEG_RGB1_X0, 0);
    dw_blk(D, sv::K3_X0 + 32, SEG_RGB1_X0, 32);
    dw_blk(D, sv::K3_X1, SEG_RGB1_X1, 0);
  }
  {
    const Geo g = geo_for_units(N);
    const int smode = scatter_mode(ns, stream);
    a.dfs = smode != 0 ? b.dfs : nullptr;
    RDRF_LAUNCH("dyn_heads_bwd", (k_dyn_density_bwd<0, false>), dim3(g.grid), dim3(g.block), stream, a, w, gw);
    if (smode != 0) {
      const int set_mask = ((g_sigma != nullptr || g_weight != nullptr) ? 1 : 0) | (g_blending != nullptr ? 2 : 0);
      if (set_mask != 0) {
        rdrf_prof_begin("scatter_dyn_density", stream);
        rc = scatter_dyn_density_sorted(a, b, P, G, set_mask, stream);
        rdrf_prof_end("scatter_dyn_density", stream);
        if (rc) return rc;
      }
    } else {
      const bool has_d = g_sigma != nullptr || g_weight != nullptr, has_b = g_blending != nullptr;
      if (has_d || has_b) {
        ScatterArgs sa;
        fill_scatter_common(sa, a);
        sa.nsets = 0;
        if (has_d) { sa.vm[sa.nsets] = P->density; sa.gvm[sa.nsets] = G->density; sa.row0[sa.nsets] = sv::K1G_DFD; ++sa.nsets; }
        if (has_b) { sa.vm[sa.nsets] = P->blending; sa.gvm[sa.nsets] = G->blending; sa.row0[sa.nsets] = sv::K1G_DFB; ++sa.nsets; }
        sa.rows = b.grows1; sa.stride = sv::K1G_ROWS;
        sa.xw = a.sp.xw;
        sa.dxw = b.dxw; sa.dxw_accumulate = 1;
        { int rc_ = launch_scatter("scatter_dyn_density", k_scatter<4, 1, 9>, sa, (long)t1, stream); if (rc_) return rc_; }
      }
    }
    RDRF_LAUNCH("dyn_warp_bwd", (k_dyn_density_bwd<1, false>), dim3(g.grid), dim3(g.block), stream, a, w, gw);
    RDRF_LAUNCH("time_branch_bwd", k_time_branch_bwd, dim3((N + TB_RPB - 1) / TB_RPB), dim3(128), stream, ts, w,
                N, b.dtout, G->l1w, G->l1b, G->l2w, G->l2b);
    const bool small_in_kernel = a.small_dw != 0;
    add_density_phase_dw(D, b.grows1, a.sp.act1, G, (int)t1, g_sigma != nullptr || g_weight != nullptr, g_blending != nullptr,
                         small_in_kernel);
  }
  rc = dw_launch(D, stream, "dw_dyn");
  return rc;
}

struct FeatWs {
  float *pk, *grows3, *grows1, *dxw, *dxn, *dtout, *gpad, *xpad;
  uint8_t* valid;
};
static int carve_feat_bwd(FeatWs& b, void* ws, size_t ws_bytes, int M, int dynamic) {
  WsCarver c(ws, ws_bytes);
  const size_t t = ((size_t)M + 31) / 32, mp = t * 32;
  b.pk = c.take<float>(PACK_AREA_FLOATS);
  b.grows3 = c.take<float>(t * sv::K3G_ROWS * 32);
  b.grows1 = dynamic ? c.take<float>(t * sv::K1G_ROWS * 32) : nullptr;
  b.dxw = dynamic ? c.take<float>(mp * 3) : nullptr;
  b.dxn = dynamic ? c.take<float>(mp * 3) : nullptr;
  b.dtout = dynamic ? c.take<float>(mp * 32) : nullptr;
  b.gpad = dynamic ? nullptr : c.take<float>(mp);
  b.xpad = dynamic ? nullptr : c.take<float>(mp * 3);
  b.valid = c.take<uint8_t>(mp);
  RDRF_CHECK(c.ok(), -3, "features backward: workspace too small: need %zu have %zu", c.off, ws_bytes);
  return 0;
}
extern "C" size_t rdrf_features_bwd_workspace_bytes(int M) {
  const size_t t = ((size_t)M + 31) / 32, mp = t * 32;
  return (size_t)PACK_AREA_FLOATS * 4 + t * (sv::K3G_ROWS + sv::K1G_ROWS) * 32 * 4 + mp * (6 + 32 + 4) * 4 + mp +
         (1 << 14);
}

extern "C" int rdrf_static_features_bwd(const RdrfStaticParams* P, const RdrfFieldCfg* cfg, const float* xn,
                                        int M, const float* g_density, const float* g_app,
                                        const RdrfStaticParams* G, float* g_xn, void* saved, size_t saved_bytes,
                                        void* ws, size_t ws_bytes, rdrf_stream_t stream_) {
  hipStream_t stream = (hipStream_t)stream_;
  if (M == 0) return 0;
  RDRF_CHECK(P && cfg && G && xn && M > 0 && (g_density || g_app), -1, "static_features_bwd: bad arguments");
  RDRF_CHECK(g_app == nullptr || saved != nullptr, -1, "static_features_bwd: the appearance features need the "
             "saved buffer of their forward call");
  const int Np = (M + 31) / 32;
  const size_t mp = (size_t)Np * 32;
  FeatWs b;
  int rc = carve_feat_bwd(b, ws, ws_bytes, M, 0);
  if (rc) return rc;
  BwdArgs a;
  fill_bwd_common(a, cfg, nullptr, nullptr, xn, nullptr, b.valid, Np, 32);
  a.M = M; a.in_norm = 1; a.g_feat = g_app; a.pk = b.pk; a.grows3 = b.grows3;
  if (saved != nullptr)
    RDRF_CHECK(carve_saved_feat(a.sp, saved, saved_bytes, 0, M), -3, "static_features_bwd: saved buffer too small");
  RDRF_FILL(b.valid, 0, mp, stream);
  RDRF_FILL(b.valid, 1, (size_t)M, stream);
  RDRF_FILL(b.xpad, 0, mp * 3 * 4, stream);
  RDRF_HIP(hipMemcpyAsync(b.xpad, xn, (size_t)M * 3 * 4, hipMemcpyDeviceToDevice, stream));
  ScatterArgs sa0;
  fill_scatter_common(sa0, a);
  sa0.xw = b.xpad;
  sa0.box.inv[0] = sa0.box.inv[1] = sa0.box.inv[2] = 1.0f;
  sa0.g_xyz = g_xn;
  if (g_density != nullptr) {
    RDRF_FILL(b.gpad, 0, mp * 4, stream);
    RDRF_HIP(hipMemcpyAsync(b.gpad, g_density, (size_t)M * 4, hipMemcpyDeviceToDevice, stream));
    ScatterArgs sa = sa0;
    sa.vm[0] = P->density; sa.gvm[0] = G->density; sa.nsets = 1;
    sa.rows = b.gpad; sa.stride = 1; sa.row0[0] = 0; sa.bcast = 1;
    { int rc_ = launch_scatter("feat_scatter_static_density", k_scatter<4, 1, 3>, sa, (long)Np, stream); if (rc_) return rc_; }
  }
  if (g_app != nullptr) {
    StaticW w;
    fill_static_w(w, P);
    StaticG gw;
    gw.density = G->density; gw.app = G->app; gw.b3 = G->b3; gw.w3 = G->w3;
    if (P->packed_bwd != nullptr) a.pk = P->packed_bwd;
    else {
      PackJobs J;
      static_pack_jobs_bwd(J, P, cfg->static_head);
      rc = pack_launch(J, b.pk, stream);
      if (rc) return rc;
    }
    const Geo g = geo_for_units(Np);
    RDRF_LAUNCH("feat_static_app_bwd", (k_static_app_bwd<RDRF_HEAD_MLP_FEA, true>), dim3(g.grid), dim3(g.block),
                stream, a, w, gw);
    ScatterArgs sa = sa0;
    sa.vm[0] = P->app; sa.gvm[0] = G->app; sa.nsets = 1;
    sa.rows = b.grows3; sa.stride = sv::K3G_ROWS; sa.row0[0] = sv::K3G_DA;
    { int rc_ = launch_scatter("feat_scatter_static_app", k_scatter<12, 3, 9>, sa, (long)Np, stream); if (rc_) return rc_; }
    DwJobs D;
    D.n = 0;
    dw_add(D, b.grows3, sv::K3G_ROWS, sv::K3G_DF, 1, 27, 0, a.sp.act3, sv::S3_ROWS, 72, 72, G->basis, nullptr,
           nullptr, Np);
    for (int i = 0; i < 3; ++i) dw_blk(D, sv::S3_G + 32 * i, SEG_IDENT, 32 * i);
    rc = dw_launch(D, stream, "feat_dw_static");
    if (rc) return rc;
  }
  return 0;
}

extern "C" int rdrf_dynamic_features_bwd(const RdrfDynamicParams* P, const RdrfFieldCfg* cfg, const float* x,
                                         const float* t, int M, int x_is_normalized, const float* g_density,
                                         const float* g_blending, const float* g_app, const float* g_xyz_prime,
                                         const RdrfDynamicParams* G, float* g_x, void* saved, size_t saved_bytes,
                                         void* ws, size_t ws_bytes, rdrf_stream_t stream_) {
  hipStream_t stream = (hipStream_t)stream_;
  if (M == 0) return 0;
  RDRF_CHECK(P && cfg && G && x && t && saved && M > 0 && (g_density || g_blending || g_app || g_xyz_prime), -1,
             "dynamic_features_bwd: bad arguments");
  const int Np = (M + 31) / 32;
  const size_t mp = (size_t)Np * 32;
  FeatWs b;
  int rc = carve_feat_bwd(b, ws, ws_bytes, M, 1);
  if (rc) return rc;
  BwdArgs a;
  fill_bwd_common(a, cfg, nullptr, t, x, nullptr, b.valid, Np, 32);
  a.M = M; a.in_norm = x_is_normalized ? 1 : 0;
  a.g_sigma = g_density; a.g_blending = g_blending; a.g_feat = g_app; a.g_xyz_prime = g_xyz_prime; a.g_xyz = g_x;
  RDRF_CHECK(carve_saved_feat(a.sp, saved, saved_bytes, 1, M), -3, "dynamic_features_bwd: saved buffer too small");
  a.pk = b.pk; a.grows1 = b.grows1; a.grows3 = b.grows3; a.dxw_app = b.dxw; a.dxn_app = b.dxn; a.dtout = b.dtout;
  DynW w;
  fill_dyn_w(w, P);
  DynG gw;
  gw.density = G->density; gw.blending = G->blending; gw.app = G->app;
  gw.rbv = G->rbv; gw.rwv = G->rwv; gw.l5b = G->l5b; gw.db2 = G->db2; gw.bb2 = G->bb2;
  gw.l5w = G->l5w; gw.dw2 = G->dw2; gw.bw2 = G->bw2;
  if (P->packed_bwd != nullptr) a.pk = P->packed_bwd;
  else {
    PackJobs J;
    dyn_pack_jobs_bwd(J, P);
    rc = pack_launch(J, b.pk, stream);
    if (rc) return rc;
  }
  RDRF_FILL(b.valid, 0, mp, stream);
  RDRF_FILL(b.valid, 1, (size_t)M, stream);
  RDRF_FILL(b.dxw, 0, mp * 3 * 4, stream);
  RDRF_FILL(b.dxn, 0, mp * 3 * 4, stream);
  const Geo g = geo_for_units(Np);
  DwJobs D;
  D.n = 0;
  if (g_app != nullptr) {
    RDRF_LAUNCH("feat_dyn_app_bwd", k_dyn_app_bwd<true>, dim3(g.grid), dim3(g.block), stream, a, w, gw);
    ScatterArgs sa;
    fill_scatter_common(sa, a);
    sa.vm[0] = P->app; sa.gvm[0] = G->app; sa.nsets = 1;
    sa.rows = b.grows3; sa.stride = sv::K3G_ROWS; sa.row0[0] = sv::K3G_DA;
    sa.xw = a.sp.xw;
    sa.dxw = b.dxw; sa.dxw_accumulate = 0;
    { int rc_ = launch_scatter("feat_scatter_dyn_app", k_scatter<12, 3, 27>, sa, (long)Np, stream); if (rc_) return rc_; }
    dw_add(D, b.grows3, sv::K3G_ROWS, sv::K3G_DF, 1, 27, 0, a.sp.act3, sv::K3_ROWS, 216, 216, G->basis, nullptr,
           nullptr, Np);
    for (int i = 0; i < 7; ++i) dw_blk(D, sv::K3_A + 32 * i, SEG_IDENT, 32 * i);
  }
  RDRF_LAUNCH("feat_dyn_heads_bwd", (k_dyn_density_bwd<0, true>), dim3(g.grid), dim3(g.block), stream, a, w, gw);
  if (g_density != nullptr || g_blending != nullptr) {
    ScatterArgs sa;
    fill_scatter_common(sa, a);
    sa.nsets = 0;
    if (g_density != nullptr) { sa.vm[sa.nsets] = P->density; sa.gvm[sa.nsets] = G->density; sa.row0[sa.nsets] = sv::K1G_DFD; ++sa.nsets; }
    if (g_blending != nullptr) { sa.vm[sa.nsets] = P->blending; sa.gvm[sa.nsets] = G->blending; sa.row0[sa.nsets] = sv::K1G_DFB; ++sa.nsets; }
    sa.rows = b.grows1; sa.stride = sv::K1G_ROWS;
    sa.xw = a.sp.xw;
    sa.dxw = b.dxw; sa.dxw_accumulate = 1;
    { int rc_ = launch_scatter("feat_scatter_dyn_density", k_scatter<4, 1, 9>, sa, (long)Np, stream); if (rc_) return rc_; }
  }
  RDRF_LAUNCH("feat_dyn_warp_bwd", (k_dyn_density_bwd<1, true>), dim3(g.grid), dim3(g.block), stream, a, w, gw);
  RDRF_LAUNCH("time_branch_bwd", k_time_branch_bwd, dim3((M + TB_RPB - 1) / TB_RPB), dim3(128), stream, t, w, M,
              b.dtout, G->l1w, G->l1b, G->l2w, G->l2b);
  add_density_phase_dw(D, b.grows1, a.sp.act1, G, Np, g_density != nullptr, g_blending != nullptr);
  return dw_launch(D, stream, "feat_dw_dyn");
}

extern "C" int rdrf_scene_flow_bwd(const RdrfDynamicParams* P, const RdrfFieldCfg* cfg,
                                   const float* pts, const float* ts, int N, int S,
                                   const float* g_sf_f, const float* g_sf_b,
                                   const RdrfDynamicParams* G, float* g_pts, void* saved,
                                   size_t saved_bytes, void* ws, size_t ws_bytes,
                                   rdrf_stream_t stream_) {
  hipStream_t stream = (hipStream_t)stream_;
  if (N == 0) return 0;
  RDRF_CHECK(P && cfg && G && saved && N > 0 && S > 0, -1, "scene_flow_bwd: bad arguments");
  RDRF_CHECK((size_t)N * S * 3 < (size_t)INT32_MAX, -1, "scene_flow_bwd: N * S * 3 must stay below 2^31 (32-bit sample indices)");
  const size_t tiles = ((size_t)N * S + 31) / 32;
  RDRF_CHECK(saved_bytes >= tiles * sv::SF_ROWS * 32 * 4, -3, "scene_flow_bwd: saved buffer too small");
  WsCarver c(ws, ws_bytes);
  float* pkbuf = c.take<float>(PACK_AREA_FLOATS);
  float* grows = c.take<float>(tiles * sv::SFG_ROWS * 32);
  RDRF_CHECK(c.ok(), -3, "scene_flow_bwd: workspace too small: need %zu have %zu", c.off, ws_bytes);
  const float* pkimg = pkbuf;
  int rc = 0;
  if (P->packed_bwd != nullptr) pkimg = P->packed_bwd;
  else {
    PackJobs J;
    dyn_pack_jobs_bwd(J, P);
    rc = pack_launch(J, pkbuf, stream);
    if (rc) return rc;
  }
  const Geo g = geo_for_units((long)tiles);
  RDRF_LAUNCH("scene_flow_bwd", k_scene_flow_bwd, dim3(g.grid), dim3(g.block), stream, N, S,
              make_box(cfg), pkimg, (const float*)saved, grows, g_sf_f, g_sf_b, G->sfb[3], g_pts);
  const float* act = (const float*)saved;
  const int T = (int)tiles;
  DwJobs D;
  D.n = 0;
  dw_add(D, grows, sv::SFG_ROWS, sv::SFG_DZ6, 1, 6, 0, act, sv::SF_ROWS, 64, 64, G->sfw[3], G->sfb[3],
         nullptr, T);
  dw_blk(D, sv::SF_H4, SEG_IDENT, 0);
  dw_blk(D, sv::SF_H4 + 32, SEG_IDENT, 32);
  dw_add(D, grows, sv::SFG_ROWS, sv::SFG_DZ4, 2, 64, 0, act, sv::SF_ROWS, 64, 64, G->sfw[2], G->sfb[2],
         nullptr, T);
  dw_blk(D, sv::SF_H2, SEG_IDENT, 0);
  dw_blk(D, sv::SF_H2 + 32, SEG_IDENT, 32);
  dw_add(D, grows, sv::SFG_ROWS, sv::SFG_DZ2, 2, 64, 0, act, sv::SF_ROWS, 64, 64, G->sfw[1], G->sfb[1],
         nullptr, T);
  dw_blk(D, sv::SF_H0, SEG_IDENT, 0);
  dw_blk(D, sv::SF_H0 + 32, SEG_IDENT, 32);
  dw_add(D, grows, sv::SFG_ROWS, sv::SFG_DZ0, 2, 64, 0, act, sv::SF_ROWS, 36, 36, G->sfw[0], G->sfb[0],
         nullptr, T);
  dw_blk(D, sv::SF_X, SEG_SF_X, 0);
  dw_blk(D, sv::SF_X + 32, SEG_SF_X, 32);
  return dw_launch(D, stream, "dw_sf");
}

#define GRB_LDS_POSES 448
__global__ __launch_bounds__(256) void k_generate_rays_bwd(const int64_t* __restrict__ ids, const float* __restrict__ uv, int view_shift,
                                    const float* __restrict__ poses9,
                                    const float* __restrict__ focal_p, int N, int T, int H, int W,
                                    int ndc, float near, const float* __restrict__ g_rays,
                                    float* __restrict__ g_poses, float* __restrict__ g_focal) {
  __shared__ float s_gp[GRB_LDS_POSES * 9];
  __shared__ float s_gf[4];
  const bool in_lds = T <= GRB_LDS_POSES;
  if (in_lds) {
    for (int i = threadIdx.x; i < T * 9; i += blockDim.x) s_gp[i] = 0.f;
    __syncthreads();
  }
  const int n = blockIdx.x * blockDim.x + threadIdx.x;
  float gf = 0.f;
  if (n < N) {
    const long id = ids[n];
    const int col = (int)(id % W), row = (int)((id / W) % H);
    int view = (int)(id / ((long)W * H)) + view_shift;
    view = view < 0 ? 0 : (view >= T ? T - 1 : view);
    const float f = focal_p[0];
    const float pu = uv ? uv[2 * n] : (float)col + 0.5f, pv = uv ? uv[2 * n + 1] : (float)row + 0.5f;
    const float dir[3] = {(pu - 0.5f * W) / f, -(pv - 0.5f * H) / f, -1.0f};
    const float* p = poses9 + view * 9;
    float b1[3] = {p[0], p[1], p[2]};
    const float n1 = sqrtf(b1[0] * b1[0] + b1[1] * b1[1] + b1[2] * b1[2]);
    for (int k = 0; k < 3; ++k) b1[k] /= n1;
    const float dt = b1[0] * p[3] + b1[1] * p[4] + b1[2] * p[5];
// ... 157 lines not shown
```

robust-dynrf_amd/csrc/rdrf_fwd.hip:

```cpp
#include "rdrf_fwd_dev.hpp"

template <bool FEAT>
__global__ __launch_bounds__(256) __attribute__((amdgpu_waves_per_eu(5, 8))) void k_static_density(FieldArgs a, StaticW w) { static_density_body<FEAT>(a, w, grid_ctx()); }

template <int HEAD, bool FEAT, bool SAVE = true>
__global__ __launch_bounds__(64 * RDRF_MAXW) void k_static_app(FieldArgs a, StaticW w) {
  static_app_body<HEAD, FEAT, SAVE>(a, w, nullptr, grid_ctx());
}

#ifdef RDRF_TOOLS
template <int HEAD, bool SAVE>
__global__ __launch_bounds__(1024) void k_static_app16(FieldArgs a, StaticW w) { static_app16_body<HEAD, SAVE>(a, w); }
#endif

template <bool FEAT, bool SAVE = true>
__global__ __launch_bounds__(64 * RDRF_MAXW) void k_dyn_density(FieldArgs a, DynW w) {
  dyn_density_body<FEAT, SAVE>(a, w, nullptr, grid_ctx());
}

template <bool FEAT, bool SAVE = true>
__global__ __launch_bounds__(64 * RDRF_MAXW) void k_dyn_app(FieldArgs a, DynW w) {
  dyn_app_body<FEAT, SAVE>(a, w, nullptr, grid_ctx());
}

__global__ __launch_bounds__(256) void k_time_branch(const float* __restrict__ ts, DynW w, int N,
                                                     float* __restrict__ tout, int* __restrict__ zero64) {
  __shared__ float s_h[8 * 64];
  if (zero64 != nullptr && blockIdx.x == 0 && threadIdx.x < 64) zero64[threadIdx.x] = 0;
  time_branch_body(ts, w, N, tout, s_h, grid_ctx());
}

__global__ __launch_bounds__(64 * RDRF_MAXW) void k_dyn_density_flat(FieldArgs a, DynW w) {
  dyn_density_body<false, false, false, true>(a, w, nullptr, grid_ctx());
}
__global__ __launch_bounds__(512) void k_ray_scan(FieldArgs a) { ray_scan_body(a); }

RDRF_D void fill_sf_x(float (&X)[20], float xn0, float xn1, float xn2, float t, int h) {
#pragma unroll
  for (int o = 0; o < 5; ++o) {
    if (o == 0 && h == 0) {
      X[0] = xn0; X[1] = xn1; X[2] = xn2; X[3] = t;
    } else {
      const int k = 2 * o + h - 1;
#pragma unroll
      for (int p = 0; p < 2; ++p) {
        const int pr = 2 * k + p;
        float sv = 0.f, cv = 0.f;
        if (pr < 16) {
          const int d = pr >> 2, f = pr & 3;
          const float x = pr < 12 ? (d == 0 ? xn0 : (d == 1 ? xn1 : xn2)) : t;
          const float a_ = ldexpf(x, f);
          if (__builtin_expect(!(fabsf(a_) <= RDRF_PE_FAST_MAX), 0)) sincosf(a_, &sv, &cv);
          else sincos_sel<true>(a_, sv, cv);
        }
        X[o * 4 + 2 * p] = sv;
        X[o * 4 + 2 * p + 1] = cv;
      }
    }
  }
}

__global__ __launch_bounds__(64 * RDRF_MAXW) void k_scene_flow(const float* __restrict__ pts,
                                                   const float* __restrict__ ts, int N, int S,
                                                   Box box, const float* __restrict__ pkg, DynW w,
                                                   float* __restrict__ sf_f,
                                                   float* __restrict__ sf_b,
                                                   float* __restrict__ act_rows, int dynq) {
  __shared__ __attribute__((aligned(16))) float lds[pk::SF_SIZE];
  __shared__ int s_next;
  if (threadIdx.x == 0) s_next = blockDim.x >> 6;
  lds_fill(lds, pkg + pk::REG_SF, pk::SF_SIZE);
  const int lane = threadIdx.x & 63, h = lane >> 5, s = lane & 31;
  const int wave = threadIdx.x >> 6, nwaves = blockDim.x >> 6;
  const float* pkw = lds;
  const int total = N * S;
  const int ntiles = (total + 31) >> 5;
  for (int k = wave, tile; (tile = blockIdx.x + k * gridDim.x) < ntiles; k = tile_queue_next(&s_next, k, nwaves, dynq != 0)) {
    const int li = tile * 32 + s;
    const bool act = li < total;
    const int idx = act ? li : 0;
    const float t = ts[idx / S];
    const float xn0 = norm_c(pts[(size_t)idx * 3 + 0], box.lo[0], box.inv[0]);
    const float xn1 = norm_c(pts[(size_t)idx * 3 + 1], box.lo[1], box.inv[1]);
    const float xn2 = norm_c(pts[(size_t)idx * 3 + 2], box.lo[2], box.inv[2]);
    float X[20];
    fill_sf_x(X, xn0, xn1, xn2, t, h);
    float* svb = act_rows ? act_rows + (size_t)tile * sv::SF_ROWS * 32 : nullptr;
    save_rows<20>(svb, sv::SF_X, X, s, h);
    f32x16 acc[2];
    acc_bias<2>(acc, pkw + pk::SF_B0, h);
    mfma_seg<2, 20>(acc, X, pkw + pk::SF_W0, lane);
    float H[32];
    acc_relu<2>(H, acc);
    save_rows<32>(svb, sv::SF_H0, H, s, h);
    acc_bias<2>(acc, pkw + pk::SF_B2, h);
    mfma_seg<2, 32>(acc, H, pkw + pk::SF_W2, lane);
    acc_relu<2>(H, acc);
    save_rows<32>(svb, sv::SF_H2, H, s, h);
    acc_bias<2>(acc, pkw + pk::SF_B4, h);
    mfma_seg<2, 32>(acc, H, pkw + pk::SF_W4, lane);
    acc_relu<2>(H, acc);
    save_rows<32>(svb, sv::SF_H4, H, s, h);
#pragma unroll
    for (int o = 0; o < 6; ++o) {
      const float v = dot_small<32>(H, pkw + pk::SF_W6 + o * 64, h) + w.sfb6[o];
      if (act && h == 0) {
        if (o < 3) sf_f[(size_t)idx * 3 + o] = v;
        else sf_b[(size_t)idx * 3 + (o - 3)] = v;
      }
    }
  }
}

void fill_common(FieldArgs& a, const RdrfFieldCfg* cfg, const float* rays, const float* ts,
                        const float* xyz, const float* z, const uint8_t* valid, int N, int S) {
  memset(&a, 0, sizeof(a));
// ... 192 lines not shown
             "static_fwd: only density comps {16,4,4} / app comps {48,12,12}, the planes and lines of a set spanning one grid, are built");
  FieldArgs a;
  fill_common(a, cfg, rays, ts, xyz, z, valid, N, S);
  a.rgb = rgb; a.sigma = sigma; a.weight = weight; a.dists = dists;
  int rc = ws_carve_fwd(a, ws, ws_bytes, N, S, saved, saved_bytes, 0);
  if (rc) return rc;
  StaticW w;
  fill_static_w(w, P);
  if (P->packed_fwd != nullptr) a.pk = P->packed_fwd;
  else {
    PackJobs J;
    static_pack_jobs_fwd(J, P, cfg->static_head);
    rc = pack_launch(J, (float*)a.pk, stream);
    if (rc) return rc;
  }
  RDRF_FILL(a.counter, 0, 256, stream);
#ifdef RDRF_DETERMINISTIC
  RDRF_FILL(a.list, 0x7f, (size_t)N * S * sizeof(int), stream);
#endif
  RDRF_LAUNCH("static_density", k_static_density<false>, dim3((N + 3) / 4), dim3(256), stream, a, w);
  if (rgb == nullptr) return 0;
#ifdef RDRF_DETERMINISTIC
  { int rc_ = rdrf_sort_ints_inplace(a.list, (unsigned)((size_t)N * S), stream); if (rc_) return rc_; }
#endif
  const Geo g = geo_for_tiles(N, S);
  const bool fea = cfg->static_head == RDRF_HEAD_MLP_FEA;
  a.dynq = fwd_dynq();
#ifdef RDRF_TOOLS
  static const int sa16 = RDRF_ENV("RDRF_SA16") ? atoi(RDRF_ENV("RDRF_SA16")) : 0;
  if (sa16) {
    const long t16 = (((long)N * S + 31) / 32) * 2;
    int waves = (int)((t16 + 255) / 256);
    waves = waves < 1 ? 1 : (waves > 16 ? 16 : waves);
    const long blocks = (t16 + waves - 1) / waves;
    const dim3 gr((unsigned)(blocks > 256 ? 256 : blocks)), bl(waves * 64);
    if (saved != nullptr) {
      if (fea) RDRF_LAUNCH("static_app", (k_static_app16<RDRF_HEAD_MLP_FEA, true>), gr, bl, stream, a, w);
      else RDRF_LAUNCH("static_app", (k_static_app16<RDRF_HEAD_MLP_FEA_TIMEEMBEDDING, true>), gr, bl, stream, a, w);
    } else {
      if (fea) RDRF_LAUNCH("static_app", (k_static_app16<RDRF_HEAD_MLP_FEA, false>), gr, bl, stream, a, w);
      else RDRF_LAUNCH("static_app", (k_static_app16<RDRF_HEAD_MLP_FEA_TIMEEMBEDDING, false>), gr, bl, stream, a, w);
    }
    return 0;
  }
#endif
  if (saved != nullptr) {
    if (fea) RDRF_LAUNCH("static_app", (k_static_app<RDRF_HEAD_MLP_FEA, false, true>), dim3(g.grid), dim3(g.block), stream, a, w);
    else RDRF_LAUNCH("static_app", (k_static_app<RDRF_HEAD_MLP_FEA_TIMEEMBEDDING, false, true>), dim3(g.grid), dim3(g.block), stream, a, w);
  } else {
    if (fea) RDRF_LAUNCH("static_app", (k_static_app<RDRF_HEAD_MLP_FEA, false, false>), dim3(g.grid), dim3(g.block), stream, a, w);
    else RDRF_LAUNCH("static_app", (k_static_app<RDRF_HEAD_MLP_FEA_TIMEEMBEDDING, false, false>), dim3(g.grid), dim3(g.block), stream, a, w);
  }
  return 0;
}

extern "C" int rdrf_dynamic_fwd(const RdrfDynamicParams* P, const RdrfFieldCfg* cfg,
                                const float* rays, const float* ts, const float* xyz,
                                const float* z, const uint8_t* valid, int N, int S,
                                float* blending, float* weight, float* xyz_prime, float* rgb,
                                float* sigma, float* dists, void* saved, size_t saved_bytes,
                                void* ws, size_t ws_bytes, rdrf_stream_t stream_) {
  hipStream_t stream = (hipStream_t)stream_;
  if (N == 0) return 0;
  RDRF_CHECK(P && cfg && N > 0 && S > 0, -1, "dynamic_fwd: bad arguments");
  RDRF_CHECK((size_t)N * S * 3 < (size_t)INT32_MAX, -1, "dynamic_fwd: N * S * 3 must stay below 2^31 (32-bit sample indices): render / train in smaller chunks");
  RDRF_CHECK(vm_ok(P->density, 16, 4) && vm_ok(P->blending, 16, 4) && vm_ok(P->app, 48, 12) && vm_same_grid(P->density, P->blending), -1,
             "dynamic_fwd: only density comps {16,4,4} / app comps {48,12,12}, the planes and lines of a set spanning one grid, are built");
  FieldArgs a;
  fill_common(a, cfg, rays, ts, xyz, z, valid, N, S);
  a.rgb = rgb; a.sigma = sigma; a.weight = weight; a.dists = dists;
  a.blending = blending; a.xyz_prime = xyz_prime;
  a.dynq = fwd_dynq();
  int rc = ws_carve_fwd(a, ws, ws_bytes, N, S, saved, saved_bytes, 1);
  if (rc) return rc;
  DynW w;
  fill_dyn_w(w, P);
  if (P->packed_fwd != nullptr) a.pk = P->packed_fwd;
  else {
    PackJobs J;
    dyn_pack_jobs_fwd(J, P);
    rc = pack_launch(J, (float*)a.pk, stream);
    if (rc) return rc;
  }
  static const int flat_env = RDRF_ENV("RDRF_FLAT") ? atoi(RDRF_ENV("RDRF_FLAT")) : 1;
  const bool flat = saved == nullptr && flat_env != 0;
  if (!flat && rgb != nullptr) RDRF_FILL(rgb, 0, (size_t)N * S * 3 * sizeof(float), stream);
  RDRF_LAUNCH("time_branch", k_time_branch, dim3((N + 7) / 8), dim3(256), stream, ts, w, N, a.tout, a.counter);
  const Geo g1 = geo_for_units(N), g3 = geo_for_tiles(N, S);
#ifdef RDRF_DETERMINISTIC
  RDRF_FILL(a.list, 0x7f, (size_t)N * S * sizeof(int), stream);
#endif
  if (saved != nullptr) RDRF_LAUNCH("dyn_density", (k_dyn_density<false, true>), dim3(g1.grid), dim3(g1.block), stream, a, w);
  else if (flat) {
    RDRF_LAUNCH("dyn_density", k_dyn_density_flat, dim3(g3.grid), dim3(g3.block), stream, a, w);
    RDRF_LAUNCH("ray_scan", k_ray_scan, dim3((N + 15) / 16), dim3(512), stream, a);
  } else RDRF_LAUNCH("dyn_density", (k_dyn_density<false, false>), dim3(g1.grid), dim3(g1.block), stream, a, w);
#ifdef RDRF_DETERMINISTIC
  { int rc_ = rdrf_sort_ints_inplace(a.list, (unsigned)((size_t)N * S), stream); if (rc_) return rc_; }
#endif
  if (rgb == nullptr) return 0;
  if (saved != nullptr) RDRF_LAUNCH("dyn_app", (k_dyn_app<false, true>), dim3(g3.grid), dim3(g3.block), stream, a, w);
  else RDRF_LAUNCH("dyn_app", (k_dyn_app<false, false>), dim3(g3.grid), dim3(g3.block), stream, a, w);
  return 0;
}

extern "C" size_t rdrf_features_saved_bytes(int dynamic, int M) { return saved_bytes_feat(dynamic, M); }
extern "C" size_t rdrf_features_workspace_bytes(int M) {
  const int Np = (M + 31) / 32;
  return rdrf_workspace_bytes(Np, 32) + (size_t)Np * 32 * (32 * 4 + 27 * 4 + 8) + (1 << 14);
}

static int feat_carve_fwd(FieldArgs& a, void* ws, size_t ws_bytes, int M, void* saved, size_t saved_bytes,
                          int dynamic) {
  WsCarver c(ws, ws_bytes);
  const size_t mp = ((size_t)M + 31) / 32 * 32;
  a.pk = c.take<float>(PACK_AREA_FLOATS);
  a.tout = c.take<float>(mp * 32);
  a.xw = c.take<float>(mp * 3);
  RDRF_CHECK(c.ok(), -3, "features: workspace too small: need %zu have %zu", c.off, ws_bytes);
  if (saved != nullptr) {
    SavedPtrs sp;
    RDRF_CHECK(carve_saved_feat(sp, saved, saved_bytes, dynamic, M), -3,
               "features: saved buffer too small: need %zu have %zu", saved_bytes_feat(dynamic, M), saved_bytes);
    a.xw = sp.xw; a.tout = sp.tout; a.raw = sp.raw; a.act1 = sp.act1; a.act3 = sp.act3;
  }
  return 0;
}

extern "C" int rdrf_static_features_fwd(const RdrfStaticParams* P, const RdrfFieldCfg* cfg, const float* xn,
                                        int M, float* density, float* app, void* saved, size_t saved_bytes,
                                        void* ws, size_t ws_bytes, rdrf_stream_t stream_) {
  hipStream_t stream = (hipStream_t)stream_;
  if (M == 0) return 0;
  RDRF_CHECK(P && cfg && xn && M > 0 && (density || app), -1, "static_features_fwd: bad arguments");
  RDRF_CHECK(vm_ok(P->density, 16, 4) && vm_ok(P->app, 48, 12), -1,
             "static_features_fwd: only density comps {16,4,4} / app comps {48,12,12}, the planes and lines of a set spanning one grid, are built");
  const int Np = (M + 31) / 32;
  FieldArgs a;
  fill_common(a, cfg, nullptr, nullptr, xn, nullptr, nullptr, Np, 32);
  a.M = M; a.in_norm = 1; a.sigma = density; a.feat = app;
  int rc = feat_carve_fwd(a, ws, ws_bytes, M, saved, saved_bytes, 0);
  if (rc) return rc;
  StaticW w;
  fill_static_w(w, P);
  if (density != nullptr)
    RDRF_LAUNCH("feat_static_density", k_static_density<true>, dim3(Np), dim3(64), stream, a, w);
  if (app != nullptr) {
    if (P->packed_fwd != nullptr) a.pk = P->packed_fwd;
    else {
      PackJobs J;
      static_pack_jobs_fwd(J, P, cfg->static_head);
      rc = pack_launch(J, (float*)a.pk, stream);
      if (rc) return rc;
    }
    const Geo g = geo_for_units(Np);
    RDRF_LAUNCH("feat_static_app", (k_static_app<RDRF_HEAD_MLP_FEA, true>), dim3(g.grid), dim3(g.block), stream,
                a, w);
  }
  return 0;
}

extern "C" int rdrf_dynamic_features_fwd(const RdrfDynamicParams* P, const RdrfFieldCfg* cfg, const float* x,
                                         const float* t, int M, int x_is_normalized, float* density,
                                         float* blending, float* app, float* xyz_prime, void* saved,
                                         size_t saved_bytes, void* ws, size_t ws_bytes,
                                         rdrf_stream_t stream_) {
  hipStream_t stream = (hipStream_t)stream_;
  if (M == 0) return 0;
  RDRF_CHECK(P && cfg && x && t && M > 0 && (density || blending || app || xyz_prime), -1,
             "dynamic_features_fwd: bad arguments");
  RDRF_CHECK(vm_ok(P->density, 16, 4) && vm_ok(P->blending, 16, 4) && vm_ok(P->app, 48, 12) && vm_same_grid(P->density, P->blending), -1,
             "dynamic_features_fwd: only density comps {16,4,4} / app comps {48,12,12}, the planes and lines of a set spanning one grid, are built");
  const int Np = (M + 31) / 32;
  FieldArgs a;
  fill_common(a, cfg, nullptr, t, x, nullptr, nullptr, Np, 32);
  a.M = M; a.in_norm = x_is_normalized ? 1 : 0;
  a.sigma = density; a.blending = blending; a.feat = app; a.xyz_prime = xyz_prime;
  int rc = feat_carve_fwd(a, ws, ws_bytes, M, saved, saved_bytes, 1);
  if (rc) return rc;
// ... 45 lines not shown
```

robust-dynrf_amd/csrc/rdrf_fwd_dev.hpp:

```cpp
#pragma once
#include "rdrf_kernels.hpp"

struct GridCtx {
  int bid, nblk, tid, nthr;
};
RDRF_D GridCtx grid_ctx() { return GridCtx{(int)blockIdx.x, (int)gridDim.x, (int)threadIdx.x, (int)blockDim.x}; }
#define GC_BID (FUSED ? gc.bid : (int)blockIdx.x)
#define GC_NBLK (FUSED ? gc.nblk : (int)gridDim.x)
#define GC_TID (FUSED ? gc.tid : (int)threadIdx.x)
#define GC_NTHR (FUSED ? gc.nthr : (int)blockDim.x)

RDRF_D int block_append_base(int* counter, int cnt, int* s_cnt, int tid, int nthr) {
  const int wave = tid >> 6, nwaves = nthr >> 6;
  __syncthreads();
  if ((tid & 63) == 0) s_cnt[wave] = cnt;
  __syncthreads();
  if (tid == 0) {
    int tot = 0;
    for (int w = 0; w < nwaves; ++w) {
      const int c = s_cnt[w];
      s_cnt[w] = tot;
      tot += c;
    }
    const int b = tot ? atomicAdd(counter, tot) : 0;
// ... 301 lines not shown
      for (int nb = 0; nb < 2; ++nb) {
        F[nb * 4 + 0] = accF[nb].x; F[nb * 4 + 1] = accF[nb].y; F[nb * 4 + 2] = accF[nb].z; F[nb * 4 + 3] = accF[nb].w;
      }
    }
    float P[32];
    {
      float fmax_ = 0.f;
#pragma unroll
      for (int r = 0; r < 8; ++r) fmax_ = fmaxf(fmax_, fabsf(F[r]));
      if (__builtin_expect(__any(!(fmax_ * 2.0f <= RDRF_PE_FAST_MAX)), 0)) {
#pragma unroll
        for (int r = 0; r < 8; ++r) {
          float s1, c1, s2, c2;
          sincosf(F[r], &s1, &c1);
          sincosf(F[r] * 2.0f, &s2, &c2);
          P[4 * r + 0] = s1; P[4 * r + 1] = c1; P[4 * r + 2] = s2; P[4 * r + 3] = c2;
        }
      } else {
#pragma unroll
        for (int r = 0; r < 8; ++r) {
          float s1, c1, s2, c2;
          sincos_sel<true>(F[r], s1, c1);
          sincos_double(s1, c1, s2, c2);
          P[4 * r + 0] = s1; P[4 * r + 1] = c1; P[4 * r + 2] = s2; P[4 * r + 3] = c2;
        }
      }
    }
    if (HEAD == RDRF_HEAD_MLP_FEA) {
      if (g == 2) F[7] = vx;
      if (g == 3) { F[4] = vy; F[5] = vz; }
    }
    if (svb != nullptr) {
      if (g == 0) {
        svb[(size_t)(sv::S3_VD + 0) * 32 + s] = vx; svb[(size_t)(sv::S3_VD + 1) * 32 + s] = vy;
        svb[(size_t)(sv::S3_VD + 2) * 32 + s] = vz;
      }
      save_rows16<8>(svb, sv::S3_F, F, voff);
#pragma unroll
      for (int r = 0; r < 8; ++r)
#pragma unroll
        for (int m = 0; m < 4; ++m)
          __builtin_nontemporal_store(P[4 * r + m], svb + (sv::S3_P + 64 * (r >> 2) + 8 * (r & 3) + m) * 32 + voffP);
    }
    f32x4 acc[8];
    float H[32];
    __builtin_amdgcn_sched_barrier(0);
    acc16_bias<8>(acc, pkw + pk::S16_B1, g);
    mfma16_seg<8, 8>(acc, F, pkw + pk::S16_W1_F, lane);
    mfma16_seg<8, 32>(acc, P, pkw + pk::S16_W1_P, lane);
    acc16_relu<8>(H, acc);
    save_rows16<32>(svb, sv::S3_H1, H, voff);
    acc16_bias<8>(acc, pkw + pk::S16_B2, g);
    mfma16_seg<8, 32>(acc, H, pkw + pk::S16_W2, lane);
    acc16_relu<8>(H, acc);
    save_rows16<32>(svb, sv::S3_H2, H, voff);
#pragma unroll
    for (int o = 0; o < 3; ++o) {
      float v = dot_small16<32>(H, pkw + pk::S16_W3 + o * 128, g) + w.b3[o];
      if (HEAD == RDRF_HEAD_MLP_FEA_TIMEEMBEDDING)
        v += w.w3[o * 131 + 128] * vx + w.w3[o * 131 + 129] * vy + w.w3[o * 131 + 130] * vz;
      if (act && g == 0) a.rgb[(size_t)idx * 3 + o] = sigmoidf_(v);
    }
  }
}

#ifndef RDRF_HEADS_F32
RDRF_D void head_layer1(f32x16 (&acc)[2], const float (&Fv)[36], const float (&X0)[32], const float (&X1)[8],
                        const float* __restrict__ wb3, const float* __restrict__ wtail, int lane) {
  float U[pk::K1_HEAD_KK];
#pragma unroll
  for (int i = 0; i < 36; ++i) U[i] = Fv[i];
#pragma unroll
  for (int i = 0; i < 32; ++i) U[36 + i] = X0[i];
#pragma unroll
  for (int i = 0; i < 4; ++i) U[68 + i] = X1[i];
  mfma_seg_b3<2, pk::K1_HEAD_KK>(acc, U, wb3, lane);
  const float V[4] = {X1[4], X1[5], X1[6], X1[7]};
  mfma_seg<2, 4>(acc, V, wtail, lane);
}
#endif

template <bool FEAT, bool SAVE = true, bool FUSED = false, bool FLAT = false>
RDRF_D void dyn_density_body(const FieldArgs a, const DynW w, float* lds_fused, const GridCtx gc) {
  static_assert(!FLAT || (!FEAT && !SAVE && !FUSED), "the flat-tile form is the inference kernel");
  float* lds;
  if constexpr (FUSED) lds = lds_fused;
  else {
    __shared__ __attribute__((aligned(16))) float lds_own[pk::K1_SIZE];
    lds = lds_own;
  }
  lds_fill(lds, a.pk + pk::REG_K1, pk::K1_SIZE);
  const int lane = GC_TID & 63, h = lane >> 5, s = lane & 31;
  const int wave = GC_TID >> 6, nwaves = GC_NTHR >> 6;
  const float* pkw = lds;
  const int nunits = FLAT ? (int)(((long)a.N * a.S + 31) >> 5) : a.N;
  for (int n = GC_BID * nwaves + wave; n < nunits; n += GC_NBLK * nwaves) {
  float t = 0.f, nrm = 1.0f;
  float T[16];
  float X1[8];
  if constexpr (!FEAT && !FLAT) {
    t = a.ts[n];
    float vx, vy, vz;
    nrm = ray_norm(a.rays, n, a.ray_type, vx, vy, vz);
#pragma unroll
    for (int q = 0; q < 4; ++q) {
      f32x4 v = ld4(a.tout + n * 32 + 8 * q + 4 * h);
      T[q * 4 + 0] = v.x; T[q * 4 + 1] = v.y; T[q * 4 + 2] = v.z; T[q * 4 + 3] = v.w;
    }
    fill_x1(X1, t, h);
  }
  float carry = 1.0f;
  int nmask = 0;
  for (int j0 = 0; j0 < (FLAT ? 32 : a.S); j0 += 32) {
    const int j = j0 + s;
    bool act;
    int idx;
    if constexpr (FLAT) {
      const long i = (long)n * 32 + s;
      act = i < (long)a.N * a.S;
      idx = act ? (int)i : 0;
    } else {
      act = j < a.S && (!FEAT || n * a.S + j < a.M);
      idx = n * a.S + (act ? j : 0);
    }
    const bool vld = act && (FEAT || a.valid[idx] != 0);
    if constexpr (FEAT || FLAT) {
      const int ti = FLAT ? idx / a.S : idx;
      t = a.ts[ti];
#pragma unroll
      for (int q = 0; q < 4; ++q) {
        f32x4 v = ld4(a.tout + (size_t)ti * 32 + 8 * q + 4 * h);
        T[q * 4 + 0] = v.x; T[q * 4 + 1] = v.y; T[q * 4 + 2] = v.z; T[q * 4 + 3] = v.w;
      }
      fill_x1(X1, t, h);
    }
#ifndef RDRF_T_RESIDENT
    if constexpr (!FEAT && !FLAT) {
      int nn = n;
      asm volatile("" : "+v"(nn));
#pragma unroll
      for (int q = 0; q < 4; ++q) {
        f32x4 v = ld4(a.tout + nn * 32 + 8 * q + 4 * h);
        T[q * 4 + 0] = v.x; T[q * 4 + 1] = v.y; T[q * 4 + 2] = v.z; T[q * 4 + 3] = v.w;
      }
    }
#endif
    const float px = a.xyz[idx * 3 + 0], py = a.xyz[idx * 3 + 1], pz = a.xyz[idx * 3 + 2];
    const bool raw_in = FEAT && a.in_norm;
    const float xn0 = raw_in ? px : norm_c(px, a.box.lo[0], a.box.inv[0]);
    const float xn1 = raw_in ? py : norm_c(py, a.box.lo[1], a.box.inv[1]);
    const float xn2 = raw_in ? pz : norm_c(pz, a.box.lo[2], a.box.inv[2]);
    float X0[32];
    fill_x0(X0, xn0, xn1, xn2, t, h);
    float* svb = (SAVE && a.act1) ? a.act1 + ((size_t)n * ((a.S + 31) >> 5) + (j0 >> 5)) * sv::K1_ROWS * 32 : nullptr;
    save_rows<32>(svb, sv::K1_X0, X0, s, h);
    save_rows<8>(svb, sv::K1_X1, X1, s, h);
    save_rows<16>(svb, sv::K1_T, T, s, h);
    float d0, d1, d2;
    {
      f32x16 acc[2];
      acc_bias<2>(acc, pkw + pk::K1_B3, h);
      mfma_seg<2, 32>(acc, X0, pkw + pk::K1_W3_X0, lane);
      mfma_seg<2, 16>(acc, T, pkw + pk::K1_W3_T, lane);
      float H3[32];
      acc_relu<2>(H3, acc);
      save_rows<32>(svb, sv::K1_H3, H3, s, h);
      acc_bias<2>(acc, pkw + pk::K1_B4, h);
      mfma_seg<2, 32>(acc, H3, pkw + pk::K1_W4, lane);
      acc_relu<2>(H3, acc);
      save_rows<32>(svb, sv::K1_H4, H3, s, h);
      d0 = dot_small<32>(H3, pkw + pk::K1_W5 + 0 * 64, h) + w.l5b[0];
      d1 = dot_small<32>(H3, pkw + pk::K1_W5 + 1 * 64, h) + w.l5b[1];
      d2 = dot_small<32>(H3, pkw + pk::K1_W5 + 2 * 64, h) + w.l5b[2];
    }
    const float xw0 = norm_c(unnorm_c(xn0, a.box.lo[0], a.box.inv[0]) + d0, a.box.lo[0], a.box.inv[0]);
    const float xw1 = norm_c(unnorm_c(xn1, a.box.lo[1], a.box.inv[1]) + d1, a.box.lo[1], a.box.inv[1]);
    const float xw2 = norm_c(unnorm_c(xn2, a.box.lo[2], a.box.inv[2]) + d2, a.box.lo[2], a.box.inv[2]);
    if (act && h == 0) {
      if (!FEAT || a.xyz_prime != nullptr) {
        a.xyz_prime[(size_t)idx * 3 + 0] = (raw_in ? unnorm_c(xn0, a.box.lo[0], a.box.inv[0]) : px) + d0;
        a.xyz_prime[(size_t)idx * 3 + 1] = (raw_in ? unnorm_c(xn1, a.box.lo[1], a.box.inv[1]) : py) + d1;
        a.xyz_prime[(size_t)idx * 3 + 2] = (raw_in ? unnorm_c(xn2, a.box.lo[2], a.box.inv[2]) : pz) + d2;
      }
      a.xw[(size_t)idx * 3 + 0] = xw0;
      a.xw[(size_t)idx * 3 + 1] = xw1;
      a.xw[(size_t)idx * 3 + 2] = xw2;
    }
    float fd, fb;
    {
      float Fv[36];
      gather_level_den<0>(w.density, point_taps(w.density, xw0, xw1, xw2, 0), h, Fv);
      gather_level_den<12>(w.density, point_taps(w.density, xw0, xw1, xw2, 1), h, Fv);
      gather_level_den<24>(w.density, point_taps(w.density, xw0, xw1, xw2, 2), h, Fv);
      if (!vld) {
#pragma unroll
        for (int i = 0; i < 36; ++i) Fv[i] = 0.f;
      }
      f32x16 acc[2];
      acc_bias<2>(acc, pkw + pk::K1_BD1, h);
#ifdef RDRF_HEADS_F32
      mfma_seg<2, 36>(acc, Fv, pkw + pk::K1_DEN1_F, lane);
      mfma_seg<2, 32>(acc, X0, pkw + pk::K1_DEN1_X0, lane);
      mfma_seg<2, 8>(acc, X1, pkw + pk::K1_DEN1_X1, lane);
#else
      head_layer1(acc, Fv, X0, X1, pkw + pk::K1_DEN1, pkw + pk::K1_DEN1_X1T, lane);
#endif
      float Hd[32];
      acc_relu<2>(Hd, acc);
      save_rows<36>(svb, sv::K1_FD, Fv, s, h);
      save_rows<32>(svb, sv::K1_HD, Hd, s, h);
      fd = dot_small<32>(Hd, pkw + pk::K1_DEN2, h) + w.db2[0];
    }
    {
      float Fv[36];
      gather_level_den<0>(w.blending, point_taps(w.blending, xw0, xw1, xw2, 0), h, Fv);
      gather_level_den<12>(w.blending, point_taps(w.blending, xw0, xw1, xw2, 1), h, Fv);
      gather_level_den<24>(w.blending, point_taps(w.blending, xw0, xw1, xw2, 2), h, Fv);
      if (!vld) {
#pragma unroll
        for (int i = 0; i < 36; ++i) Fv[i] = 0.f;
      }
      f32x16 acc[2];
      acc_bias<2>(acc, pkw + pk::K1_BB1, h);
#ifdef RDRF_HEADS_F32
      mfma_seg<2, 36>(acc, Fv, pkw + pk::K1_BLE1_F, lane);
      mfma_seg<2, 32>(acc, X0, pkw + pk::K1_BLE1_X0, lane);
      mfma_seg<2, 8>(acc, X1, pkw + pk::K1_BLE1_X1, lane);
#else
      head_layer1(acc, Fv, X0, X1, pkw + pk::K1_BLE1, pkw + pk::K1_BLE1_X1T, lane);
#endif
      float Hd[32];
      acc_relu<2>(Hd, acc);
      save_rows<36>(svb, sv::K1_FB, Fv, s, h);
      save_rows<32>(svb, sv::K1_HB, Hd, s, h);
      fb = dot_small<32>(Hd, pkw + pk::K1_BLE2, h) + w.bb2[0];
    }
    if constexpr (FEAT) {
      if (act && h == 0) {
        if (a.sigma != nullptr) a.sigma[idx] = fd;
        if (a.blending != nullptr) a.blending[idx] = fb;
        if (a.raw != nullptr) { a.raw[(size_t)idx * 2] = fd; a.raw[(size_t)idx * 2 + 1] = fb; }
      }
    } else if constexpr (FLAT) {
      if (act && h == 0) {
        a.sigma[idx] = vld ? density_act(fd, a.act, a.density_shift) : 0.0f;
        a.blending[idx] = vld ? sigmoidf_(fb) : 0.0f;
      }
    } else {
    const float sigma = vld ? density_act(fd, a.act, a.density_shift) : 0.0f;
    const float blend = vld ? sigmoidf_(fb) : 0.0f;
    const float zj = act ? a.z[idx] : 0.f;
    const float zn = (j + 1 < a.S) ? a.z[idx + 1] : zj;
    const float ds = ((j + 1 < a.S) ? (zn - zj) : 0.0f) * nrm * a.distance_scale;
    const float alpha = 1.0f - expf(-sigma * ds);
    const float p = act ? one_minus_alpha_eps(alpha) : 1.0f;
    const float incl = scan_mul32(p, s);
    float excl = __shfl_up(incl, 1, 32);
    if (s == 0) excl = 1.0f;
    const float Tr = carry * excl;
    const float wt = alpha * Tr;
    carry *= __shfl(incl, 31, 32);
    const bool m = act && h == 0 && wt > a.weight_thres;
    if (act && h == 0) {
      a.sigma[idx] = sigma;
      a.weight[idx] = wt;
      a.dists[idx] = ds;
      a.blending[idx] = blend;
      if (SAVE && a.raw != nullptr) { a.raw[(size_t)idx * 2] = fd; a.raw[(size_t)idx * 2 + 1] = fb; }
    }
    nmask += __popcll(__ballot(m));
    }
  }
  if constexpr (!FEAT && !FLAT) {
    if (nmask) {
      int base = 0;
      if (lane == 0) base = atomicAdd(a.counter, nmask);
      base = __shfl(base, 0, 64);
      for (int j0 = 0; j0 < a.S; j0 += 32) {
        const int j = j0 + s;
        const bool act = j < a.S && h == 0;
        const int idx = n * a.S + (act ? j : 0);
        const bool m = act && a.weight[idx] > a.weight_thres;
        const unsigned long long bal = __ballot(m);
        if (m) a.list[base + __builtin_amdgcn_mbcnt_hi((unsigned)(bal >> 32), __builtin_amdgcn_mbcnt_lo((unsigned)bal, 0u))] = idx;
        base += __popcll(bal);
      }
    }
  }
  }
}

RDRF_D void ray_scan_body(const FieldArgs a) {
  __shared__ int s_cnt[16];
  const int lane = threadIdx.x & 63, h = lane >> 5, s = lane & 31;
  const int n_ = (blockIdx.x * (blockDim.x >> 6) + (threadIdx.x >> 6)) * 2 + h;
  const bool ray = n_ < a.N;
  const int n = ray ? n_ : 0;
  float vx, vy, vz;
  const float nrm = ray_norm(a.rays, n, a.ray_type, vx, vy, vz);
  float carry = 1.0f;
  int cnt = 0;
  for (int j0 = 0; j0 < a.S; j0 += 32) {
    const int j = j0 + s;
    const bool act = ray && j < a.S;
    const int idx = n * a.S + (act ? j : 0);
    const float sigma = act ? a.sigma[idx] : 0.0f;
    const float zj = act ? a.z[idx] : 0.f;
    const float zn = (j + 1 < a.S) ? a.z[idx + 1] : zj;
    const float ds = ((j + 1 < a.S) ? (zn - zj) : 0.0f) * nrm * a.distance_scale;
    const float alpha = 1.0f - expf(-sigma * ds);
    const float p = act ? one_minus_alpha_eps(alpha) : 1.0f;
    const float incl = scan_mul32(p, s);
    float excl = __shfl_up(incl, 1, 32);
    if (s == 0) excl = 1.0f;
    const float Tr = carry * excl;
    const float wt = alpha * Tr;
    carry *= __shfl(incl, 31, 32);
    if (act) {
      a.weight[idx] = wt;
      a.dists[idx] = ds;
    }
    if (ray && a.rgb != nullptr) {
      float* r = a.rgb + ((size_t)n * a.S + j0) * 3 + s;
      const int lim = (a.S - j0 < 32 ? a.S - j0 : 32) * 3;
      if (s < lim) r[0] = 0.f;
      if (s + 32 < lim) r[32] = 0.f;
      if (s + 64 < lim) r[64] = 0.f;
    }
    cnt += __popcll(__ballot(act && wt > a.weight_thres));
// ... 177 lines not shown
```

robust-dynrf_amd/csrc/rdrf_host.hpp:

```cpp
#pragma once
#include <hip/hip_runtime.h>
#include <stdarg.h>
#include <stdio.h>
#include <stdlib.h>
#include <string.h>

#include "rdrf_common.hpp"

void rdrf_set_error(const char* fmt, ...);

#ifdef RDRF_TOOLS
#include <stdlib.h>
#define RDRF_ENV(name) getenv(name)
#else
#define RDRF_ENV(name) ((const char*)nullptr)
#endif

#define RDRF_CHECK(cond, code, ...)  \
  do {                               \
    if (!(cond)) {                   \
      rdrf_set_error(__VA_ARGS__);   \
      return (code);                 \
    }                                \
  } while (0)

#define RDRF_HIP(expr)                                                             \
  do {                                                                             \
    hipError_t e_ = (expr);                                                        \
    if (e_ != hipSuccess) {                                                        \
      rdrf_set_error("%s failed: %s (%s:%d)", #expr, hipGetErrorString(e_), __FILE__, __LINE__); \
      return -5;                                                                   \
    }                                                                              \
  } while (0)

int rdrf_fill_async(void* p, int byte_value, size_t bytes, hipStream_t stream);
#define RDRF_FILL(p, v, bytes, stream)                          \
  do {                                                          \
    int rc_fill_ = rdrf_fill_async((p), (v), (bytes), (stream)); \
    if (rc_fill_) return rc_fill_;                              \
  } while (0)

void rdrf_prof_begin(const char* name, hipStream_t s);
void rdrf_prof_end(const char* name, hipStream_t s);

#define RDRF_LAUNCH(name, kernel, grid, block, stream, ...)            \
  do {                                                                 \
    rdrf_prof_begin(name, stream);                                     \
    hipLaunchKernelGGL(kernel, grid, block, 0, stream, __VA_ARGS__);   \
    rdrf_prof_end(name, stream);                                       \
    RDRF_HIP(hipGetLastError());                                       \
  } while (0)

static inline Box make_box(const RdrfFieldCfg* cfg) {
  Box b;
  for (int i = 0; i < 3; ++i) {
    b.lo[i] = cfg->aabb[i];
    b.hi[i] = cfg->aabb[3 + i];
    b.inv[i] = 2.0f / (cfg->aabb[3 + i] - cfg->aabb[i]);
  }
  return b;
}

struct WsCarver {
  char* base;
  size_t off, cap;
  WsCarver(void* p, size_t c) : base((char*)p), off(0), cap(c) {}
  template <typename T>
  T* take(size_t n) {
    size_t bytes = (n * sizeof(T) + 255) & ~(size_t)255;
    T* r = (T*)(base + off);
    off += bytes;
    return r;
  }
  bool ok() const { return off <= cap; }
};

static inline bool vm_one_grid(const RdrfVM& v) {
  return v.W[0] == v.W[1] && v.W[0] == v.L[2] && v.H[0] == v.W[2] && v.H[0] == v.L[1] && v.H[1] == v.H[2] && v.H[1] == v.L[0];
}
static inline bool vm_same_grid(const RdrfVM& a, const RdrfVM& b) {
  return a.W[0] == b.W[0] && a.H[0] == b.H[0] && a.L[0] == b.L[0];
}
static inline bool vm_ok(const RdrfVM& v, int c0, int c1) {
  return v.C[0] == c0 && v.C[1] == c1 && v.C[2] == c1 && vm_one_grid(v);
}

size_t rdrf_sort_temp_bytes(unsigned n, int bits);
int rdrf_sort_positions(const unsigned* keys_in, unsigned* keys_out, unsigned* vals_out, unsigned n, int bits, void* temp,
                        size_t temp_bytes, hipStream_t stream, const int* n_dev = nullptr, unsigned n_mul = 0);

int rdrf_sort_ints_inplace(int* data, unsigned n, hipStream_t stream);

void pack_add(PackJobs& J, const float* src, int ld, int out_dim, int in_dim, int seg, int mode,
              int nb, int kk, int dst);
void pack_add_b3(PackJobs& J, const float* src, int ld, int out_dim, int in_dim, int seg, int nb, int kk, int seg_kk0, int kk_off,
                 int kk_tot, int dst);
void pack_add_b3s(PackJobs& J, const float* src, int ld, int out_dim, int in_dim, int seg, int nb, int kk, int seg_kk0, int kk_off,
                  int kk_tot, int dst, int dst_lo);
void pack_add_b3s_t(PackJobs& J, const float* src, int ld, int out_dim, int in_dim, int seg, int nbi, int kk, int dst, int dst_lo);
// ... 3 lines not shown
```

Baseline: 425,200 rays/s.

## Use flat sample-tile layout for dynamic density in training forward and backward

Extends the flat tile form of the dynamic density kernel, which packs samples from consecutive rays into 32-wide tiles with no per-ray padding, from inference to the training path. The forward pass now saves activations and raw outputs in the flat layout, with a dynamic tile queue. The backward pass gains a separate per-ray scan kernel that computes sigma gradients into a new buffer. The density backward and scatter kernels then run over flat tiles, and partial time-branch gradients for rays that straddle tiles go to a separate buffer. This removes padding waste when S=115 does not divide by 32, at the cost of an extra scan kernel, more workspace and segmented reductions.

```diff
diff --git a/robust-dynrf_amd/csrc/rdrf_bwd.hip b/robust-dynrf_amd/csrc/rdrf_bwd.hip
--- a/robust-dynrf_amd/csrc/rdrf_bwd.hip
+++ b/robust-dynrf_amd/csrc/rdrf_bwd.hip
@@ -100,6 +100,8 @@
   float* dxw_app;
   float* dxn_app;
   float* dtout;
+  float* gsig;
+  float* dtp;
   float* dfs;
   float* dfa;
   float* g_xyz;
@@ -1034,6 +1036,7 @@
   RdrfVM vm[2], gvm[2];
   int nsets;
   const float* rows;
+  int flat;
   int stride, row0[2];
   const float* xw;
   const float* xyz;
@@ -1062,7 +1065,7 @@
   const int wave = threadIdx.x >> 6, nwaves = blockDim.x >> 6;
   const int tpr = (a.S + 31) >> 5;
   const int count = a.list ? *a.count : 0;
-  const int ntiles = a.list ? ((count + 31) >> 5) : a.N * tpr;
+  const int ntiles = a.list ? ((count + 31) >> 5) : (a.flat ? (a.N * a.S + 31) >> 5 : a.N * tpr);
   for (int t = blockIdx.x * nwaves + wave; t < ntiles; t += gridDim.x * nwaves) {
     int idx;
     bool live;
@@ -1070,6 +1073,11 @@
       const int li = t * 32 + s;
       live = li < count;
       idx = live ? a.list[li] : 0;
+    } else if (a.flat) {
+      const int i = t * 32 + s;
+      const bool act = i < a.N * a.S;
+      idx = act ? i : 0;
+      live = act && a.valid[idx] != 0;
     } else {
       const int n = t / tpr, j = (t - n * tpr) * 32 + s;
       const bool act = j < a.S;
@@ -1172,6 +1180,7 @@
   int kb;
   unsigned* keys;
   int* counts;
+  int flat;
   int compact;
 };
 
@@ -1195,7 +1204,8 @@
     } else {
       const int idx = e;
       const int n = idx / a.S, j = idx - n * a.S;
-      const float* sm = a.grows1 + ((size_t)(n * tpr + (j >> 5)) * sv::K1G_ROWS + sv::K1G_SM) * 32 + (j & 31);
+      const float* sm = a.grows1 + ((size_t)(a.flat ? idx >> 5 : n * tpr + (j >> 5)) * sv::K1G_ROWS + sv::K1G_SM) * 32 +
+                        (a.flat ? idx & 31 : j & 31);
       live = a.valid[idx] != 0 && (sm[3 * 32] != 0.f || sm[4 * 32] != 0.f);
       x0 = a.xw[(size_t)idx * 3 + 0]; x1 = a.xw[(size_t)idx * 3 + 1]; x2 = a.xw[(size_t)idx * 3 + 2];
     }
@@ -1434,8 +1444,86 @@
   return (b0 ? u[1] : u[0]) + __shfl_xor(b0 ? u[0] : u[1], 1, 64);
 }
 
-template <int PHASE, bool FEAT>
+__global__ __launch_bounds__(512) void k_ray_scan_bwd(BwdArgs a) {
+  __shared__ float carr[16][128];
+  const int lane = threadIdx.x & 63, h = lane >> 5, s = lane & 31;
+  const int hw = (threadIdx.x >> 6) * 2 + h;
+  const int n_ = blockIdx.x * 16 + hw;
+  const bool ray = n_ < a.N;
+  const int n = ray ? n_ : 0;
+  const int tpr = (a.S + 31) >> 5;
+  float vx, vy, vz;
+  const float nrm = ray_norm(a.rays, n, a.ray_type, vx, vy, vz);
+  if (a.g_weight) {
+    float carry = 1.0f;
+    for (int j0 = 0; j0 < a.S; j0 += 32) {
+      if (s == 0) carr[hw][j0 >> 5] = carry;
+      const int j = j0 + s;
+      const bool act = ray && j < a.S;
+      const int idx = n * a.S + (act ? j : 0);
+      const bool vld = act && a.valid[idx] != 0;
+      const float sigma = vld ? density_act(a.sp.raw[(size_t)idx * 2], a.act, a.density_shift) : 0.f;
+      const float zj = act ? a.z[idx] : 0.f;
+      const float zn = (j + 1 < a.S) ? a.z[idx + 1] : zj;
+      const float ds = ((j + 1 < a.S) ? (zn - zj) : 0.0f) * nrm * a.distance_scale;
+      const float alpha = 1.0f - expf(-sigma * ds);
+      const float p = act ? one_minus_alpha_eps(alpha) : 1.0f;
+      carry *= __shfl(scan_mul32(p, s), 31, 32);
+    }
+  }
+  float sufcarry = 0.f, g_nrm = 0.f;
+  for (int tli = tpr - 1; tli >= 0; --tli) {
+    const int j = (tli << 5) + s;
+    const bool act = ray && j < a.S;
+    const int idx = n * a.S + (act ? j : 0);
+    const bool vld = act && a.valid[idx] != 0;
+    const float sigma = vld ? density_act(a.sp.raw[(size_t)idx * 2], a.act, a.density_shift) : 0.f;
+    const float zj = act ? a.z[idx] : 0.f;
+    const float zn = (j + 1 < a.S) ? a.z[idx + 1] : zj;
+    const float ds = ((j + 1 < a.S) ? (zn - zj) : 0.0f) * nrm * a.distance_scale;
+    const float alpha = 1.0f - expf(-sigma * ds);
+    const float p = act ? one_minus_alpha_eps(alpha) : 1.0f;
+    float g_alpha = 0.f;
+    if (a.g_weight) {
+      const float incl = scan_mul32(p, s);
+      float excl = __shfl_up(incl, 1, 32);
+      if (s == 0) excl = 1.0f;
+      const float T = carr[hw][tli] * excl;
+      const float gwv = act ? a.g_weight[idx] : 0.f;
+      float rinc = gwv * alpha * T;
+#pragma unroll
+      for (int d = 1; d < 32; d <<= 1) {
+        const float o = __shfl_down(rinc, d, 32);
+        if (s + d < 32) rinc += o;
+      }
+      float rex = __shfl_down(rinc, 1, 32);
+      if (s == 31) rex = 0.f;
+      g_alpha = gwv * T - (sufcarry + rex) / p;
+      sufcarry += __shfl(rinc, 0, 32);
+    }
+    float g_sigma = (act && a.g_sigma) ? a.g_sigma[idx] : 0.f;
+    g_sigma += g_alpha * ds * (1.0f - alpha);
+    if (act) a.gsig[idx] = g_sigma;
+    if ((a.g_rays || a.g_z) && act) {
+      const float g_ds = (a.g_dists ? a.g_dists[idx] : 0.f) + g_alpha * sigma * (1.0f - alpha);
+      if (a.g_rays) g_nrm += g_ds * ((j + 1 < a.S) ? (zn - zj) : 0.0f) * a.distance_scale;
+      if (a.g_z && j + 1 < a.S) {
+        const float gz = g_ds * nrm * a.distance_scale;
+        atomicAdd(a.g_z + idx, -gz);
+        atomicAdd(a.g_z + idx + 1, gz);
+      }
+    }
+  }
+  if (a.g_rays && a.ray_type != RDRF_RAY_OTHER) {
+#pragma unroll
+    for (int d = 16; d >= 1; d >>= 1) g_nrm += __shfl_xor(g_nrm, d, 64);
+    if (ray && s < 3) atomicAdd(a.g_rays + (size_t)n * 6 + 3 + s, g_nrm * (s == 0 ? vx : (s == 1 ? vy : vz)));
+  }
+}
+
+template <int PHASE, bool FEAT, bool FLAT = false>
 __global__ __launch_bounds__(64 * RDRF_MAXW) void k_dyn_density_bwd(BwdArgs a, DynW w, DynG gw) {
+  static_assert(!(FLAT && FEAT), "feature mode keeps its pseudo-ray geometry (S = 32: a ray is a tile)");
   __shared__ __attribute__((aligned(16))) float lds[PHASE == 0 ? pkb::K1H_SIZE : pkb::K1W_SIZE];
   __shared__ float carr[8][128];
   lds_fill(lds, a.pk + (PHASE == 0 ? pkb::REG_K1H : pkb::REG_K1W), PHASE == 0 ? pkb::K1H_SIZE : pkb::K1W_SIZE);
@@ -1443,11 +1531,12 @@
   const int wave = threadIdx.x >> 6, nwaves = blockDim.x >> 6;
   const int tpr = (a.S + 31) >> 5;
   float sw[3] = {0.f, 0.f, 0.f}, sb[3] = {0.f, 0.f, 0.f};
-  for (int n = blockIdx.x * nwaves + wave; n < a.N; n += gridDim.x * nwaves) {
+  const int nunits = FLAT ? (a.N * a.S + 31) >> 5 : a.N;
+  for (int n = blockIdx.x * nwaves + wave; n < nunits; n += gridDim.x * nwaves) {
     float vx = 0.f, vy = 0.f, vz = 0.f;
     float nrm = 1.0f;
-    if constexpr (!FEAT) nrm = ray_norm(a.rays, n, a.ray_type, vx, vy, vz);
-    if (!FEAT && PHASE == 0 && a.g_weight) {
+    if constexpr (!FEAT && !FLAT) nrm = ray_norm(a.rays, n, a.ray_type, vx, vy, vz);
+    if (!FEAT && !FLAT && PHASE == 0 && a.g_weight) {
       float carry = 1.0f;
       for (int j0 = 0; j0 < a.S; j0 += 32) {
         if (lane == 0) carr[wave][j0 >> 5] = carry;
@@ -1468,13 +1557,13 @@
     float dTacc[16];
 #pragma unroll
     for (int i = 0; i < 16; ++i) dTacc[i] = 0.f;
-    for (int tli = tpr - 1; tli >= 0; --tli) {
+    for (int tli = FLAT ? 0 : tpr - 1; tli >= 0; --tli) {
       const int j0 = tli << 5;
       const int j = j0 + s;
-      const bool act = j < a.S && (!FEAT || n * a.S + j < a.M);
-      const int idx = n * a.S + (act ? j : 0);
+      const bool act = FLAT ? n * 32 + s < a.N * a.S : j < a.S && (!FEAT || n * a.S + j < a.M);
+      const int idx = FLAT ? (act ? n * 32 + s : 0) : n * a.S + (act ? j : 0);
       const bool vld = act && (FEAT || a.valid[idx] != 0);
-      const size_t tl = (size_t)n * tpr + tli;
+      const size_t tl = FLAT ? (size_t)n : (size_t)n * tpr + tli;
       const float* svb = a.sp.act1 + tl * sv::K1_ROWS * 32;
       float* gb = a.grows1 + tl * sv::K1G_ROWS * 32;
       if (PHASE == 0) {
@@ -1482,6 +1571,12 @@
         if constexpr (FEAT) {
           g_fd = (act && a.g_sigma) ? a.g_sigma[idx] : 0.f;
           g_fb = (act && a.g_blending) ? a.g_blending[idx] : 0.f;
+        } else if constexpr (FLAT) {
+          const float fd = a.sp.raw[(size_t)idx * 2], fb = a.sp.raw[(size_t)idx * 2 + 1];
+          const float g_sigma = act ? a.gsig[idx] : 0.f;
+          g_fd = vld ? g_sigma * act_grad(fd, a.act, a.density_shift) : 0.f;
+          const float bl = sigmoidf_(fb);
+          g_fb = (vld && a.g_blending) ? a.g_blending[idx] * bl * (1.0f - bl) : 0.f;
         } else {
         const float fd = a.sp.raw[(size_t)idx * 2], fb = a.sp.raw[(size_t)idx * 2 + 1];
         const float sigma = vld ? density_act(fd, a.act, a.density_shift) : 0.f;
@@ -1693,16 +1788,34 @@
         }
       }
     }
-    if (PHASE == 1 && !FEAT) {
+    if (PHASE == 1 && !FEAT && FLAT) {
+      const int i0 = n * 32 + s, nl = i0 / a.S;
+      const int rb = nl * a.S - n * 32, re = rb + a.S - 1;
+      const int end = re < 31 ? re : 31;
+      const bool head = i0 < a.N * a.S && (s == 0 || rb == s);
+      float* dst = (rb >= 0 && re <= 31) ? a.dtout + (size_t)nl * 32
+                                         : a.dtp + ((size_t)n * 2 + (s == 0 ? 0 : 1)) * 32;
 #pragma unroll
       for (int i = 0; i < 16; ++i) {
         float v = dTacc[i];
 #pragma unroll
+        for (int d = 1; d < 32; d <<= 1) {
+          const float o = __shfl_down(v, d, 32);
+          if (s + d <= end) v += o;
+        }
+        if (head) dst[elem_of(i, h)] = v;
+      }
+    }
+    if (PHASE == 1 && !FEAT && !FLAT) {
+#pragma unroll
+      for (int i = 0; i < 16; ++i) {
+        float v = dTacc[i];
+#pragma unroll
         for (int d = 16; d >= 1; d >>= 1) v += __shfl_xor(v, d, 64);
         if (s == 0) a.dtout[(size_t)n * 32 + elem_of(i, h)] = v;
       }
     }
-    if (!FEAT && PHASE == 0 && a.g_rays && a.ray_type != RDRF_RAY_OTHER) {
+    if (!FEAT && !FLAT && PHASE == 0 && a.g_rays && a.ray_type != RDRF_RAY_OTHER) {
       g_nrm = wave_sum(g_nrm);
       if (lane < 3) atomicAdd(a.g_rays + (size_t)n * 6 + 3 + lane, g_nrm * (lane == 0 ? vx : (lane == 1 ? vy : vz)));
     }
@@ -1736,8 +1849,17 @@
 }
 
 #define TB_RPB 32
+RDRF_D float dtout_of_ray(const float* __restrict__ dtout, const float* __restrict__ dtp, int S, int n, int o) {
+  const int b = n * S, t0 = b >> 5, t1 = (b + S - 1) >> 5;
+  if (dtp == nullptr || t0 == t1) return dtout[(size_t)n * 32 + o];
+  float v = dtp[((size_t)t0 * 2 + ((b & 31) == 0 ? 0 : 1)) * 32 + o];
+  for (int t = t0 + 1; t <= t1; ++t) v += dtp[(size_t)t * 64 + o];
+  return v;
+}
+
 __global__ __launch_bounds__(128) void k_time_branch_bwd(const float* __restrict__ ts, DynW w, int N,
                                                          const float* __restrict__ dtout,
+                                                         const float* __restrict__ dtp, int S,
                                                          float* __restrict__ g_l1w,
                                                          float* __restrict__ g_l1b,
                                                          float* __restrict__ g_l2w,
@@ -1757,7 +1879,7 @@
   for (int f = 0; f < 8; ++f) sincosf(ldexpf(t, f), &tin[1 + f], &tin[9 + f]);
   if (q == 0)
     for (int i = 0; i < 17; ++i) s_tin[r][i] = tin[i];
-  for (int o = q; o < 30; o += 4) s_dz2[r][o] = act ? dtout[(size_t)n * 32 + o] : 0.f;
+  for (int o = q; o < 30; o += 4) s_dz2[r][o] = act ? dtout_of_ray(dtout, dtp, S, n, o) : 0.f;
   __syncthreads();
   for (int k = 16 * q; k < 16 * q + 16; ++k) {
     float hk = w.l1b[k];
@@ -2413,6 +2535,7 @@
   size_t bwd = (size_t)PACK_AREA_FLOATS * 4 + t1 * sv::K1G_ROWS * 32 * 4 + t3 * sv::K3G_ROWS * 32 * 4 +
                ns * 3 * 4 * 2 + (size_t)N * 32 * 4 + (1 << 14);
   bwd += ns * DFS_FLOATS * 4 + ns * DFA_FLOATS * 4 + 3 * ns * 4 * 3 + 1024 + rdrf_sort_temp_bytes((unsigned)(3 * ns), 32) + (1 << 12);
+  bwd += ns * 4 + t3 * 64 * 4 + 512;
   size_t sf = (size_t)PACK_AREA_FLOATS * 4 + t3 * sv::SFG_ROWS * 32 * 4 + (1 << 12);
   size_t m = fwd > bwd ? fwd : bwd;
   return m > sf ? m : sf;
@@ -2432,6 +2555,8 @@
   float* dxw;
   float* dxn;
   float* dtout;
+  float* gsig;
+  float* dtp;
 };
 static int carve_bwd(BwdWs& b, void* ws, size_t ws_bytes, int N, int S, int dynamic) {
   WsCarver c(ws, ws_bytes);
@@ -2445,6 +2570,7 @@
   b.gf = dynamic ? nullptr : c.take<float>(t1 * 32);
   b.dfs = nullptr;
   b.dfa = nullptr;
+  b.gsig = b.dtp = nullptr;
   if (dynamic) {
     b.dfs = c.take<float>(ns * DFS_FLOATS);
     b.dfa = c.take<float>(ns * DFA_FLOATS);
@@ -2454,6 +2580,8 @@
     b.counts = c.take<int>(64);
     b.sort_tmp_bytes = rdrf_sort_temp_bytes((unsigned)(3 * ns), 32);
     b.sort_tmp = c.take<char>(b.sort_tmp_bytes);
+    b.gsig = c.take<float>(ns);
+    b.dtp = c.take<float>(t3 * 64);
   }
   RDRF_CHECK(c.ok(), -3, "backward workspace too small: need %zu have %zu", c.off, ws_bytes);
   return 0;
@@ -2696,6 +2824,7 @@
   SortKeyArgs ka;
   memset(&ka, 0, sizeof(ka));
   ka.grows1 = b.grows1;
+  ka.flat = rdrf_flat_density() ? 1 : 0;
   int rc = sorted_scatter_prepare(ka, P->density, a, b, stream);
   if (rc) return rc;
   SortedScatterArgs sa;
@@ -2865,6 +2994,8 @@
   if (rc) return rc;
   a.pk = b.pk; a.grows1 = b.grows1; a.grows3 = b.grows3; a.dxw_app = b.dxw; a.dxn_app = b.dxn;
   a.dtout = b.dtout;
+  const bool flat = rdrf_flat_density();
+  a.gsig = b.gsig; a.dtp = b.dtp;
   DynW w;
   fill_dyn_w(w, P);
   DynG gw;
@@ -2878,7 +3009,7 @@
     rc = pack_launch(J, b.pk, stream);
     if (rc) return rc;
   }
-  const size_t ns = (size_t)N * S, t3 = (ns + 31) / 32, t1 = (size_t)N * ((S + 31) / 32);
+  const size_t ns = (size_t)N * S, t3 = (ns + 31) / 32, t1 = flat ? t3 : (size_t)N * ((S + 31) / 32);
   RDRF_FILL(b.dxw, 0, ns * 3 * 4, stream);
   RDRF_FILL(b.dxn, 0, ns * 3 * 4, stream);
   const int* cnt = &a.sp.hdr->count;
@@ -2922,10 +3053,13 @@
     dw_blk(D, sv::K3_X1, SEG_RGB1_X1, 0);
   }
   {
-    const Geo g = geo_for_units(N);
+    const Geo g = geo_for_units(flat ? (long)t1 : (long)N);
     const int smode = scatter_mode(ns, stream);
     a.dfs = smode != 0 ? b.dfs : nullptr;
-    RDRF_LAUNCH("dyn_heads_bwd", (k_dyn_density_bwd<0, false>), dim3(g.grid), dim3(g.block), stream, a, w, gw);
+    if (flat) {
+      RDRF_LAUNCH("ray_scan_bwd", k_ray_scan_bwd, dim3((N + 15) / 16), dim3(512), stream, a);
+      RDRF_LAUNCH("dyn_heads_bwd", (k_dyn_density_bwd<0, false, true>), dim3(g.grid), dim3(g.block), stream, a, w, gw);
+    } else RDRF_LAUNCH("dyn_heads_bwd", (k_dyn_density_bwd<0, false>), dim3(g.grid), dim3(g.block), stream, a, w, gw);
     if (smode != 0) {
       const int set_mask = ((g_sigma != nullptr || g_weight != nullptr) ? 1 : 0) | (g_blending != nullptr ? 2 : 0);
       if (set_mask != 0) {
@@ -2942,15 +3076,16 @@
         sa.nsets = 0;
         if (has_d) { sa.vm[sa.nsets] = P->density; sa.gvm[sa.nsets] = G->density; sa.row0[sa.nsets] = sv::K1G_DFD; ++sa.nsets; }
         if (has_b) { sa.vm[sa.nsets] = P->blending; sa.gvm[sa.nsets] = G->blending; sa.row0[sa.nsets] = sv::K1G_DFB; ++sa.nsets; }
-        sa.rows = b.grows1; sa.stride = sv::K1G_ROWS;
+        sa.rows = b.grows1; sa.stride = sv::K1G_ROWS; sa.flat = flat ? 1 : 0;
         sa.xw = a.sp.xw;
         sa.dxw = b.dxw; sa.dxw_accumulate = 1;
         { int rc_ = launch_scatter("scatter_dyn_density", k_scatter<4, 1, 9>, sa, (long)t1, stream); if (rc_) return rc_; }
       }
     }
-    RDRF_LAUNCH("dyn_warp_bwd", (k_dyn_density_bwd<1, false>), dim3(g.grid), dim3(g.block), stream, a, w, gw);
+    if (flat) RDRF_LAUNCH("dyn_warp_bwd", (k_dyn_density_bwd<1, false, true>), dim3(g.grid), dim3(g.block), stream, a, w, gw);
+    else RDRF_LAUNCH("dyn_warp_bwd", (k_dyn_density_bwd<1, false>), dim3(g.grid), dim3(g.block), stream, a, w, gw);
     RDRF_LAUNCH("time_branch_bwd", k_time_branch_bwd, dim3((N + TB_RPB - 1) / TB_RPB), dim3(128), stream, ts, w,
-                N, b.dtout, G->l1w, G->l1b, G->l2w, G->l2b);
+                N, b.dtout, flat ? (const float*)b.dtp : nullptr, S, G->l1w, G->l1b, G->l2w, G->l2b);
     const bool small_in_kernel = a.small_dw != 0;
     add_density_phase_dw(D, b.grows1, a.sp.act1, G, (int)t1, g_sigma != nullptr || g_weight != nullptr, g_blending != nullptr,
                          small_in_kernel);
@@ -3117,7 +3252,7 @@
   }
   RDRF_LAUNCH("feat_dyn_warp_bwd", (k_dyn_density_bwd<1, true>), dim3(g.grid), dim3(g.block), stream, a, w, gw);
   RDRF_LAUNCH("time_branch_bwd", k_time_branch_bwd, dim3((M + TB_RPB - 1) / TB_RPB), dim3(128), stream, t, w, M,
-              b.dtout, G->l1w, G->l1b, G->l2w, G->l2b);
+              b.dtout, (const float*)nullptr, 32, G->l1w, G->l1b, G->l2w, G->l2b);
   add_density_phase_dw(D, b.grows1, a.sp.act1, G, Np, g_density != nullptr, g_blending != nullptr);
   return dw_launch(D, stream, "feat_dw_dyn");
 }
diff --git a/robust-dynrf_amd/csrc/rdrf_fwd.hip b/robust-dynrf_amd/csrc/rdrf_fwd.hip
--- a/robust-dynrf_amd/csrc/rdrf_fwd.hip
+++ b/robust-dynrf_amd/csrc/rdrf_fwd.hip
@@ -30,8 +30,9 @@
   time_branch_body(ts, w, N, tout, s_h, grid_ctx());
 }
 
+template <bool SAVE>
 __global__ __launch_bounds__(64 * RDRF_MAXW) void k_dyn_density_flat(FieldArgs a, DynW w) {
-  dyn_density_body<false, false, false, true>(a, w, nullptr, grid_ctx());
+  dyn_density_body<false, SAVE, false, true>(a, w, nullptr, grid_ctx());
 }
 __global__ __launch_bounds__(512) void k_ray_scan(FieldArgs a) { ray_scan_body(a); }
 
@@ -390,19 +391,19 @@
     rc = pack_launch(J, (float*)a.pk, stream);
     if (rc) return rc;
   }
-  static const int flat_env = RDRF_ENV("RDRF_FLAT") ? atoi(RDRF_ENV("RDRF_FLAT")) : 1;
-  const bool flat = saved == nullptr && flat_env != 0;
+  const bool flat = rdrf_flat_density();
   if (!flat && rgb != nullptr) RDRF_FILL(rgb, 0, (size_t)N * S * 3 * sizeof(float), stream);
   RDRF_LAUNCH("time_branch", k_time_branch, dim3((N + 7) / 8), dim3(256), stream, ts, w, N, a.tout, a.counter);
   const Geo g1 = geo_for_units(N), g3 = geo_for_tiles(N, S);
 #ifdef RDRF_DETERMINISTIC
   RDRF_FILL(a.list, 0x7f, (size_t)N * S * sizeof(int), stream);
 #endif
-  if (saved != nullptr) RDRF_LAUNCH("dyn_density", (k_dyn_density<false, true>), dim3(g1.grid), dim3(g1.block), stream, a, w);
-  else if (flat) {
-    RDRF_LAUNCH("dyn_density", k_dyn_density_flat, dim3(g3.grid), dim3(g3.block), stream, a, w);
+  if (flat) {
+    if (saved != nullptr) RDRF_LAUNCH("dyn_density", k_dyn_density_flat<true>, dim3(g3.grid), dim3(g3.block), stream, a, w);
+    else RDRF_LAUNCH("dyn_density", k_dyn_density_flat<false>, dim3(g3.grid), dim3(g3.block), stream, a, w);
     RDRF_LAUNCH("ray_scan", k_ray_scan, dim3((N + 15) / 16), dim3(512), stream, a);
-  } else RDRF_LAUNCH("dyn_density", (k_dyn_density<false, false>), dim3(g1.grid), dim3(g1.block), stream, a, w);
+  } else if (saved != nullptr) RDRF_LAUNCH("dyn_density", (k_dyn_density<false, true>), dim3(g1.grid), dim3(g1.block), stream, a, w);
+  else RDRF_LAUNCH("dyn_density", (k_dyn_density<false, false>), dim3(g1.grid), dim3(g1.block), stream, a, w);
 #ifdef RDRF_DETERMINISTIC
   { int rc_ = rdrf_sort_ints_inplace(a.list, (unsigned)((size_t)N * S), stream); if (rc_) return rc_; }
 #endif
diff --git a/robust-dynrf_amd/csrc/rdrf_fwd_dev.hpp b/robust-dynrf_amd/csrc/rdrf_fwd_dev.hpp
--- a/robust-dynrf_amd/csrc/rdrf_fwd_dev.hpp
+++ b/robust-dynrf_amd/csrc/rdrf_fwd_dev.hpp
@@ -407,19 +407,24 @@
 
 template <bool FEAT, bool SAVE = true, bool FUSED = false, bool FLAT = false>
 RDRF_D void dyn_density_body(const FieldArgs a, const DynW w, float* lds_fused, const GridCtx gc) {
-  static_assert(!FLAT || (!FEAT && !SAVE && !FUSED), "the flat-tile form is the inference kernel");
+  static_assert(!FLAT || (!FEAT && !FUSED), "the flat-tile form is a ray-path kernel of its own");
   float* lds;
   if constexpr (FUSED) lds = lds_fused;
   else {
     __shared__ __attribute__((aligned(16))) float lds_own[pk::K1_SIZE];
     lds = lds_own;
   }
-  lds_fill(lds, a.pk + pk::REG_K1, pk::K1_SIZE);
   const int lane = GC_TID & 63, h = lane >> 5, s = lane & 31;
   const int wave = GC_TID >> 6, nwaves = GC_NTHR >> 6;
+  __shared__ int s_next;
+  if (FLAT && GC_TID == 0) s_next = nwaves;
+  lds_fill(lds, a.pk + pk::REG_K1, pk::K1_SIZE);
   const float* pkw = lds;
   const int nunits = FLAT ? (int)(((long)a.N * a.S + 31) >> 5) : a.N;
-  for (int n = GC_BID * nwaves + wave; n < nunits; n += GC_NBLK * nwaves) {
+  const bool dynq = FLAT && (a.dynq & 1) != 0;
+  int k = wave;
+  for (int n = FLAT ? GC_BID + k * GC_NBLK : GC_BID * nwaves + wave; n < nunits;
+       n = FLAT ? GC_BID + (k = tile_queue_next(&s_next, k, nwaves, dynq)) * GC_NBLK : n + GC_NBLK * nwaves) {
   float t = 0.f, nrm = 1.0f;
   float T[16];
   float X1[8];
@@ -477,7 +482,7 @@
     const float xn2 = raw_in ? pz : norm_c(pz, a.box.lo[2], a.box.inv[2]);
     float X0[32];
     fill_x0(X0, xn0, xn1, xn2, t, h);
-    float* svb = (SAVE && a.act1) ? a.act1 + ((size_t)n * ((a.S + 31) >> 5) + (j0 >> 5)) * sv::K1_ROWS * 32 : nullptr;
+    float* svb = (SAVE && a.act1) ? a.act1 + (FLAT ? (size_t)n : (size_t)n * ((a.S + 31) >> 5) + (j0 >> 5)) * sv::K1_ROWS * 32 : nullptr;
     save_rows<32>(svb, sv::K1_X0, X0, s, h);
     save_rows<8>(svb, sv::K1_X1, X1, s, h);
     save_rows<16>(svb, sv::K1_T, T, s, h);
@@ -570,6 +575,7 @@
       if (act && h == 0) {
         a.sigma[idx] = vld ? density_act(fd, a.act, a.density_shift) : 0.0f;
         a.blending[idx] = vld ? sigmoidf_(fb) : 0.0f;
+        if (SAVE && a.raw != nullptr) { a.raw[(size_t)idx * 2] = fd; a.raw[(size_t)idx * 2 + 1] = fb; }
       }
     } else {
     const float sigma = vld ? density_act(fd, a.act, a.density_shift) : 0.0f;
diff --git a/robust-dynrf_amd/csrc/rdrf_host.hpp b/robust-dynrf_amd/csrc/rdrf_host.hpp
--- a/robust-dynrf_amd/csrc/rdrf_host.hpp
+++ b/robust-dynrf_amd/csrc/rdrf_host.hpp
@@ -15,6 +15,11 @@
 #else
 #define RDRF_ENV(name) ((const char*)nullptr)
 #endif
+
+inline bool rdrf_flat_density() {
+  static const bool flat = !(RDRF_ENV("RDRF_FLAT") != nullptr && atoi(RDRF_ENV("RDRF_FLAT")) == 0);
+  return flat;
+}
 
 #define RDRF_CHECK(cond, code, ...)  \
   do {                               \
```

New measurement: 438,300 rays/s, median of 6. 1.03x the previous value.
